# zhyever/PatchFusion

Hardware: AMD Instinct MI355X
Metric: patches/sec (DepthAnything-ViT-L PatchFusion, 4K image, P=16 tiles at N=1) (higher is better)
Workload: dtype f32; 1 GPU; Depth-Anything-vitl14 PatchFusion, 2160x3840 synthetic RGB, 4x4 regular tiling (cai_mode m1, 16 tiles), process_num=8, random-init weights (BASELINE.json configs[2] at N=1; 16 tiles per GPU); parallelism=single GPU

## Files before the change

### include/pf_hip.h

```cpp
#ifndef PF_HIP_H
#define PF_HIP_H
#include <stdint.h>

#ifdef __cplusplus
extern "C" {
#endif

#define PF_DTYPE_F32 0
#define PF_DTYPE_BF16 1

#define PF_ACT_NONE 0
#define PF_ACT_RELU 1
#define PF_ACT_GELU 2
#define PF_ACT_SOFTPLUS 3

const char* pf_last_error(void);
int pf_version(void);

typedef struct {
  const void* x; int x_ld; int B, H, W, Cin;
  const void* w; int w_rows; int Kpad;
  const float* bias; const float* scale;
  const void* res; int res_ld; const void* res2; int res2_ld;
  void* y; int y_ld; int OH, OW, Cout;
  int KH, KW, stride, pad;
  int act;
  int relu_in;
  int out_f32;
  int shuffle;
  int dtype;
  int korder;
  int batch;
  long x_bstride, w_bstride, y_bstride;
  const int* col_exp;
  const int* out_exp;
} pf_conv_params;
int pf_conv(const pf_conv_params* p, void* stream);
int pf_conv_timed(const pf_conv_params* p, int iters, float* ms, void* stream);

int pf_conv_winograd(const pf_conv_params* p, int m, const void* U, int u_rows, int u_kpad, void* V, void* M, void* stream);
int pf_conv_winograd_split3(const pf_conv_params* p, const void* U3, int u_rows, int u_kpad, void* V3, void* M, void* stream);
int pf_conv_winograd_split3_windowed(const pf_conv_params* p, const void* U3, int u_rows, int u_kpad, void* V3, void* M, long window, void* stream);
long pf_wino_f16x2_scratch_bytes(int cin, int u_rows);
int pf_conv_winograd_f16x2_supported(const pf_conv_params* p, int u_rows, int u_kpad, long window);
int pf_conv_winograd_f16x2_windowed(const pf_conv_params* p, const void* U, int u_rows, int u_kpad, void* V2, void* M, void* scratch, long window,
                                    void* stream);
int pf_conv_winograd_f16x2_windowed_ex(const pf_conv_params* p, const void* U, int u_rows, int u_kpad, void* V2, void* M, void* scratch, long window,
                                       const void* cmax_in, void* cmax_out, int cmax_out_relu, void* stream);
int pf_conv_winograd_split3_windowed_ex(const pf_conv_params* p, const void* U3, int u_rows, int u_kpad, void* V3, void* M, long window, void* cmax_out,
                                        int cmax_out_relu, void* stream);
int pf_wino_absmax(const void* x, int x_ld, long P, int C, int relu_in, void* cmax, void* stream);
int pf_gemm_f16x2_points(const pf_conv_params* p, const int* col_exp, int grid_cap, void* stream);
int pf_gemm_f16x2_points128(const pf_conv_params* p, const int* col_exp, int grid_cap, void* stream);
int pf_gemm_f16x2_points_route(const pf_conv_params* p, int cus);
int pf_gemm_f16x2_points_route_ex(const pf_conv_params* p, int cus, int maxima_given);
int pf_conv_winograd_f16x2_supported_ex(const pf_conv_params* p, int u_rows, int u_kpad, long window, int maxima_given);
int pf_gemm_f16x2(const pf_conv_params* p, void* stream);

int pf_conv_winograd_fused_supported(const pf_conv_params* p);
int pf_conv_winograd_fused(const pf_conv_params* p, const void* up, int nnb, int gs, void* stream);
int pf_conv_winograd_fused_timed(const pf_conv_params* p, const void* up, int nnb, int gs, int iters, float* ms, void* stream);

int pf_gemm_split3(const pf_conv_params* p, void* stream);
int pf_conv1x1_split3(const pf_conv_params* p, const void* w3, int w3_rows, void* stream);
int pf_gemm_split3_ex(const pf_conv_params* p, int grid_cap, void* stream);
#define PF_S3_ROUTE_TILE64 0
#define PF_S3_ROUTE_TILE128 1
#define PF_S3_ROUTE_PERSIST128 2
#define PF_S3_ROUTE_PERSIST192 3
int pf_gemm_split3_route(const pf_conv_params* p, int cus);
int pf_gemm_split3_timed(const pf_conv_params* p, int iters, float* ms, void* stream);
int pf_gemm_bf16_pp(const pf_conv_params* p, void* stream);
int pf_layernorm_split3(const float* x, int x_ld, void* y3, int y_ld, long plane, int kmajor, const float* g, const float* b, float eps,
                        long rows, int D, void* stream);
int pf_layernorm_f16x2(const float* x, int x_ld, void* y2, const int* in_exp, const float* g, const float* b, float eps, long rows, int D,
                       void* stream);
int pf_vit_attention_qkv_split3(const void* qkv, void* out3, long plane, int kmajor, int B, int S, int Hh, void* stream);
int pf_vit_attention_split3(const void* qkv3, long plane_in, void* out3, long plane_out, int kmajor, int B, int S, int Hh, void* stream);
int pf_vit_attention_split3_v2(const void* qkv3, long plane_in, void* out3, long plane_out, int kmajor, int B, int S, int Hh, int queries_per_wave,
                               int schedule, void* stream);
int pf_vit_attention_f16x2(const void* qkv2, long plane_in, const int* qk_exp, void* out, long plane_out, const int* v_exp3, int B, int S, int Hh,
                           void* stream);
int pf_vit_attention_split3_rpb(const void* qkv3, long plane_in, void* out3, long plane_out, int kmajor, int B, int S, int Hh, const float* tab,
                                int th, int tw, int queries_per_wave, void* stream);
int pf_vit_attention_rpb_bf16(const void* q, const void* k, const void* vt, void* out, int B, int S, int Sp, int Hh, const float* tab, int th, int tw,
                              void* stream);
int pf_vit_attention_rpb_bf16_lds_bytes(int S, int th, int tw);
int pf_split3(const float* x, int x_ld, void* y, int y_ld, long plane, long rows, int cols, void* stream);

int pf_patch_im2col(const float* img, int B, int H, int W, void* out, int ld, int dtype, void* stream);
int pf_patch_im2col_norm(const float* img, int B, int H, int W, int patch, const float* mean3, const float* std3, float* out, int ld, void* stream);
int pf_readout_concat(const float* x, int x_ld, int B, int S, int D, float* y, int y_ld, void* stream);
int pf_patch_im2col_norm_bf16(const float* img, int B, int H, int W, int patch, const float* mean3, const float* std3, void* out, int ld, void* stream);
int pf_readout_concat_bf16(const void* x, int x_ld, int B, int S, int D, void* y, int y_ld, void* stream);
int pf_assemble_tokens(const void* emb, void* tokens, const float* cls, const float* pos, int B, int S, int D, int dtype,
                       void* stream);
int pf_layernorm(const void* x, int x_ld, void* y, int y_ld, const float* g, const float* b, float eps,
                 int batches, int in_rows_per_batch, int in_row_offset, int out_rows_per_batch, int D,
                 int dtype, void* stream);
int pf_qkv_split(const void* qkv, int B, int S, int Hh, void* q, void* k, void* vt, int Sp, float scale,
                 int dtype, void* stream);
int pf_vit_attention(const void* q, const void* k, const void* vt, void* out, int B, int S, int Sp, int Hh,
                     int dtype, void* stream);
int pf_vit_attention_qkv(const void* qkv, void* out, int B, int S, int Hh, int dtype, void* stream);

int pf_swin_ln_partition(const void* x, int x_ld, void* xw, const float* g, const float* b, float eps,
                         int B, int H, int W, int C, int shift, int dtype, void* stream);
int pf_swin_window_attention(const void* qkv, void* out, const float* bias_table, int B, int Hp, int Wp,
                             int C, int heads, int shift, int dtype, void* stream);
int pf_swin_unpartition_add(const void* proj, const void* shortcut, int s_ld, void* y, int y_ld, int B, int H,
                            int W, int C, int shift, int dtype, void* stream);
int pf_add_rowwise(void* x, int x_ld, const float* pos, int B, int T, int C, int dtype, void* stream);

int pf_resize_bilinear(const void* x, int x_ld, int B, int H, int W, int C, void* y, int y_ld, int OH, int OW,
                       const void* add, int add_ld, int in_f32, int out_f32, int dtype, void* stream);
int pf_resize_concat(const void* const* xs, const int* lds, const int* Hs, const int* Ws, const int* Cs, int nsrc, int B,
                     void* y, int y_ld, int OH, int OW, int dtype, void* stream);
int pf_crop_resize_planar(const float* img, int C, int H, int W, const int* boxes, int P, float* out, int oh, int ow,
                          void* stream);
int pf_roi_align(const void* feat, int f_ld, int Bf, int H, int W, int C, const float* rois, int K, void* y,
                 int y_ld, int oh, int ow, float spatial_scale, int in_f32, int out_f32, int dtype, void* stream);
int pf_maxpool2(const void* x, int x_ld, int B, int H, int W, int C, void* y, int y_ld, int dtype, void* stream);
int pf_copy_channels(const void* x, int x_ld, void* y, int y_ld, long npix, int C, int in_f32, int out_f32,
                     int dtype, void* stream);
int pf_zero_u32(void* p, long n, void* stream);
int pf_resize_bilinear_ex(const void* x, int x_ld, int B, int H, int W, int C, void* y, int y_ld, int OH, int OW,
                          const void* add, int add_ld, int in_f32, int out_f32, int dtype, void* cmax, void* stream);
int pf_resize_concat_ex(const void* const* xs, const int* lds, const int* Hs, const int* Ws, const int* Cs, int nsrc, int B,
                        void* y, int y_ld, int OH, int OW, int dtype, void* cmax, void* stream);
int pf_roi_align_ex(const void* feat, int f_ld, int Bf, int H, int W, int C, const float* rois, int K, void* y,
                    int y_ld, int oh, int ow, float spatial_scale, int in_f32, int out_f32, int dtype, void* cmax, void* stream);
int pf_copy_channels_ex(const void* x, int x_ld, void* y, int y_ld, long npix, int C, int in_f32, int out_f32,
                        int dtype, void* cmax, void* stream);
int pf_pack_fusion_input(const float* cdepth, const float* fdepth, const float* crops, void* y, int B, int h, int w,
                         int dtype, void* stream);
int pf_nhwc_to_nchw_f32(const void* x, int x_ld, float* y, int B, int H, int W, int C, int in_f32, int dtype, void* stream);

int pf_attractor(const float* A, int a_ld, int n_attr, int a_stride, float a_eps, int attractor_exp, int kind_sum,
                 const float* b_prev, int hp, int wp, float* out, int B, int h, int w, int n_bins, void* stream);
int pf_seed_bin_centers(const float* x, int x_ld, float* out, long npix, int n_bins, float min_depth, float max_depth, int bounded,
                        int normalize, void* stream);
int pf_bounded_bin_centers(const float* b, float* out, long npix, int n_bins, float min_depth, float max_depth, void* stream);
int pf_logbinom_depth(const float* pt, int pt_ld, const float* centers, int hc, int wc, float* depth, int B, int h,
                      int w, int n_bins, float min_temp, float max_temp, void* stream);
int pf_bins_tail(const float* clb, int clb_ld, int rel_off, const float* emb, int he, int we, const float* w0f, const float* b0,
                 const float* w2, const float* b2, const float* centers, int hc, int wc, float* depth, int B, int H, int W, int nq,
                 float min_temp, float max_temp, void* stream);

int pf_stitch_init(float* pred, float* count, int MH, int MW, const float* depth, const float* mask, const int* yx,
                   int P, int ph, int pw, void* stream);
int pf_stitch_finish_init(float* avg, const float* pred, const float* count, long n, void* stream);
int pf_stitch_update(float* avg, float* count, int MH, int MW, const float* depth, int dh, int dw, const float* mask,
                     int y0, int x0, int ph, int pw, void* stream);
int pf_resize_nearest_f32(const float* x, int H, int W, float* y, int OH, int OW, void* stream);
int pf_resize_bilinear_f32(const float* x, int H, int W, float* y, int OH, int OW, void* stream);


int pf_u8_bicubic_to_f32(const uint8_t* src, int H, int W, int reverse_channels, float* dst, int OH, int OW, void* stream);

int pf_percentile_workspace_bytes(void);
int pf_percentiles_f32(const float* x, long n, float invalid_val, int use_invalid, const uint8_t* invalid_mask, double q0, double q1,
                       float* out2, void* workspace, void* stream);

int pf_colorize_f32(const float* depth, long n, const float* vmin_vmax, const uint8_t* lut_rgba, int N, float invalid_val,
                    int use_invalid, const uint8_t* invalid_mask, uint32_t background_rgba, uint8_t* out_rgba, void* stream);

int pf_depth_to_u16(const float* depth, long n, float scale, uint16_t* out, void* stream);

int pf_depth_metrics(const float* gt, int H, int W, const float* pred, int ph, int pw, const float* edges,
                     const uint8_t* additional_mask, float min_depth, float max_depth, int crop_y0, int crop_y1, int crop_x0, int crop_x1,
                     double* out13, void* stream);

int pf_silog_loss(const float* pred, const float* target, long n, float min_depth, float max_depth, float beta, double* ws3,
                  float* loss, void* stream);

#ifdef __cplusplus
}
#endif
#endif
```

### patchfusion_amd/_lib.py

```python
import ctypes as C
import os

import torch

_HERE = os.path.dirname(os.path.abspath(__file__))
LIB_PATH = os.environ.get("PF_LIB_PATH") or os.path.join(_HERE, "libpf_hip.so")

vp, ci, cf, cl = C.c_void_p, C.c_int, C.c_float, C.c_long


class ConvParams(C.Structure):
    _fields_ = [
        ("x", vp), ("x_ld", ci), ("B", ci), ("H", ci), ("W", ci), ("Cin", ci),
        ("w", vp), ("w_rows", ci), ("Kpad", ci),
        ("bias", vp), ("scale", vp),
        ("res", vp), ("res_ld", ci), ("res2", vp), ("res2_ld", ci),
        ("y", vp), ("y_ld", ci), ("OH", ci), ("OW", ci), ("Cout", ci),
        ("KH", ci), ("KW", ci), ("stride", ci), ("pad", ci),
        ("act", ci), ("relu_in", ci), ("out_f32", ci), ("shuffle", ci), ("dtype", ci), ("korder", ci),
        ("batch", ci), ("x_bstride", C.c_long), ("w_bstride", C.c_long), ("y_bstride", C.c_long),
        ("col_exp", vp), ("out_exp", vp),
    ]


SIGNATURES = {
    "pf_conv": [C.POINTER(ConvParams), vp],
    "pf_conv_timed": [C.POINTER(ConvParams), ci, C.POINTER(cf), vp],
    "pf_patch_im2col": [vp, ci, ci, ci, vp, ci, ci, vp],
    "pf_assemble_tokens": [vp, vp, vp, vp, ci, ci, ci, ci, vp],
    "pf_layernorm": [vp, ci, vp, ci, vp, vp, cf, ci, ci, ci, ci, ci, ci, vp],
    "pf_qkv_split": [vp, ci, ci, ci, vp, vp, vp, ci, cf, ci, vp],
    "pf_vit_attention": [vp, vp, vp, vp, ci, ci, ci, ci, ci, vp],
    "pf_vit_attention_qkv": [vp, vp, ci, ci, ci, ci, vp],
    "pf_swin_ln_partition": [vp, ci, vp, vp, vp, cf, ci, ci, ci, ci, ci, ci, vp],
    "pf_swin_window_attention": [vp, vp, vp, ci, ci, ci, ci, ci, ci, ci, vp],
    "pf_swin_unpartition_add": [vp, vp, ci, vp, ci, ci, ci, ci, ci, ci, ci, vp],
    "pf_add_rowwise": [vp, ci, vp, ci, ci, ci, ci, vp],
    "pf_resize_bilinear": [vp, ci, ci, ci, ci, ci, vp, ci, ci, ci, vp, ci, ci, ci, ci, vp],
    "pf_resize_concat": [C.POINTER(vp), C.POINTER(ci), C.POINTER(ci), C.POINTER(ci), C.POINTER(ci), ci, ci, vp, ci, ci, ci, ci, vp],
    "pf_crop_resize_planar": [vp, ci, ci, ci, vp, ci, vp, ci, ci, vp],
    "pf_roi_align": [vp, ci, ci, ci, ci, ci, vp, ci, vp, ci, ci, ci, cf, ci, ci, ci, vp],
    "pf_maxpool2": [vp, ci, ci, ci, ci, ci, vp, ci, ci, vp],
    "pf_copy_channels": [vp, ci, vp, ci, cl, ci, ci, ci, ci, vp],
    "pf_resize_bilinear_ex": [vp, ci, ci, ci, ci, ci, vp, ci, ci, ci, vp, ci, ci, ci, ci, vp, vp],
    "pf_resize_concat_ex": [C.POINTER(vp), C.POINTER(ci), C.POINTER(ci), C.POINTER(ci), C.POINTER(ci), ci, ci, vp, ci, ci, ci, ci, vp, vp],
    "pf_roi_align_ex": [vp, ci, ci, ci, ci, ci, vp, ci, vp, ci, ci, ci, cf, ci, ci, ci, vp, vp],
    "pf_copy_channels_ex": [vp, ci, vp, ci, cl, ci, ci, ci, ci, vp, vp],
    "pf_zero_u32": [vp, cl, vp],
    "pf_pack_fusion_input": [vp, vp, vp, vp, ci, ci, ci, ci, vp],
    "pf_nhwc_to_nchw_f32": [vp, ci, vp, ci, ci, ci, ci, ci, ci, vp],
    "pf_conv_winograd": [C.POINTER(ConvParams), ci, vp, ci, ci, vp, vp, vp],
    "pf_conv_winograd_split3": [C.POINTER(ConvParams), vp, ci, ci, vp, vp, vp],
    "pf_conv_winograd_split3_windowed": [C.POINTER(ConvParams), vp, ci, ci, vp, vp, C.c_long, vp],
    "pf_conv_winograd_f16x2_windowed": [C.POINTER(ConvParams), vp, ci, ci, vp, vp, vp, C.c_long, vp],
    "pf_conv_winograd_f16x2_windowed_ex": [C.POINTER(ConvParams), vp, ci, ci, vp, vp, vp, C.c_long, vp, vp, ci, vp],
    "pf_conv_winograd_split3_windowed_ex": [C.POINTER(ConvParams), vp, ci, ci, vp, vp, C.c_long, vp, ci, vp],
    "pf_wino_absmax": [vp, ci, cl, ci, ci, vp, vp],
    "pf_gemm_f16x2_points": [C.POINTER(ConvParams), vp, ci, vp],
    "pf_gemm_f16x2_points128": [C.POINTER(ConvParams), vp, ci, vp],
    "pf_gemm_f16x2": [C.POINTER(ConvParams), vp],
    "pf_gemm_split3": [C.POINTER(ConvParams), vp],
    "pf_gemm_split3_ex": [C.POINTER(ConvParams), ci, vp],
    "pf_conv1x1_split3": [C.POINTER(ConvParams), vp, ci, vp],
    "pf_gemm_split3_timed": [C.POINTER(ConvParams), ci, C.POINTER(cf), vp],
    "pf_gemm_bf16_pp": [C.POINTER(ConvParams), vp],
    "pf_split3": [vp, ci, vp, ci, cl, cl, ci, vp],
    "pf_layernorm_split3": [vp, ci, vp, ci, cl, ci, vp, vp, cf, cl, ci, vp],
    "pf_layernorm_f16x2": [vp, ci, vp, vp, vp, vp, cf, cl, ci, vp],
    "pf_vit_attention_qkv_split3": [vp, vp, cl, ci, ci, ci, ci, vp],
    "pf_vit_attention_split3": [vp, cl, vp, cl, ci, ci, ci, ci, vp],
    "pf_vit_attention_split3_v2": [vp, cl, vp, cl, ci, ci, ci, ci, ci, ci, vp],
    "pf_vit_attention_f16x2": [vp, cl, vp, vp, cl, vp, ci, ci, ci, vp],
    "pf_vit_attention_split3_rpb": [vp, cl, vp, cl, ci, ci, ci, ci, vp, ci, ci, ci, vp],
    "pf_patch_im2col_norm": [vp, ci, ci, ci, ci, vp, vp, vp, ci, vp],
    "pf_readout_concat": [vp, ci, ci, ci, ci, vp, ci, vp],
    "pf_vit_attention_rpb_bf16": [vp, vp, vp, vp, ci, ci, ci, ci, vp, ci, ci, vp],
    "pf_patch_im2col_norm_bf16": [vp, ci, ci, ci, ci, vp, vp, vp, ci, vp],
    "pf_readout_concat_bf16": [vp, ci, ci, ci, ci, vp, ci, vp],
    "pf_conv_winograd_fused": [C.POINTER(ConvParams), vp, ci, ci, vp],
    "pf_conv_winograd_fused_timed": [C.POINTER(ConvParams), vp, ci, ci, ci, C.POINTER(cf), vp],
    "pf_attractor": [vp, ci, ci, ci, cf, ci, ci, vp, ci, ci, vp, ci, ci, ci, ci, vp],
    "pf_seed_bin_centers": [vp, ci, vp, cl, ci, cf, cf, ci, ci, vp],
    "pf_bounded_bin_centers": [vp, vp, cl, ci, cf, cf, vp],
    "pf_logbinom_depth": [vp, ci, vp, ci, ci, vp, ci, ci, ci, ci, cf, cf, vp],
    "pf_bins_tail": [vp, ci, ci, vp, ci, ci, vp, vp, vp, vp, vp, ci, ci, vp, ci, ci, ci, ci, cf, cf, vp],
    "pf_stitch_init": [vp, vp, ci, ci, vp, vp, vp, ci, ci, ci, vp],
    "pf_stitch_finish_init": [vp, vp, vp, cl, vp],
    "pf_stitch_update": [vp, vp, ci, ci, vp, ci, ci, vp, ci, ci, ci, ci, vp],
    "pf_resize_nearest_f32": [vp, ci, ci, vp, ci, ci, vp],
    "pf_resize_bilinear_f32": [vp, ci, ci, vp, ci, ci, vp],
    "pf_u8_bicubic_to_f32": [vp, ci, ci, ci, vp, ci, ci, vp],
    "pf_percentiles_f32": [vp, cl, cf, ci, vp, C.c_double, C.c_double, vp, vp, vp],
    "pf_colorize_f32": [vp, cl, vp, vp, ci, cf, ci, vp, C.c_uint32, vp, vp],
    "pf_depth_to_u16": [vp, cl, cf, vp, vp],
    "pf_silog_loss": [vp, vp, cl, cf, cf, cf, vp, vp, vp],
    "pf_depth_metrics": [vp, ci, ci, vp, ci, ci, vp, vp, cf, cf, ci, ci, ci, ci, vp, vp],
}
NON_STATUS = ("pf_last_error", "pf_version", "pf_percentile_workspace_bytes", "pf_conv_winograd_fused_supported", "pf_gemm_split3_route",
              "pf_gemm_f16x2_points_route", "pf_gemm_f16x2_points_route_ex", "pf_conv_winograd_f16x2_supported_ex",
              "pf_wino_f16x2_scratch_bytes", "pf_conv_winograd_f16x2_supported", "pf_vit_attention_rpb_bf16_lds_bytes")

_lib = None


def load():
    global _lib
    if _lib is not None:
        return _lib
    if not os.path.exists(LIB_PATH):
        raise ImportError(
            f"{LIB_PATH} not found: the HIP extension is not built. Run `python __graft_entry__.py` "
            "(or `make -C patchfusion_amd/csrc`). There is no CPU fallback for the product path.")
    lib = C.CDLL(LIB_PATH)
    for name, args in SIGNATURES.items():
        fn = getattr(lib, name)
        fn.argtypes = args
        fn.restype = ci
    lib.pf_last_error.restype = C.c_char_p
    lib.pf_last_error.argtypes = []
    lib.pf_version.restype = ci
    lib.pf_version.argtypes = []
    lib.pf_percentile_workspace_bytes.restype = ci
    lib.pf_percentile_workspace_bytes.argtypes = []
    lib.pf_conv_winograd_fused_supported.restype = ci
    lib.pf_conv_winograd_fused_supported.argtypes = [C.POINTER(ConvParams)]
    lib.pf_gemm_split3_route.restype = ci
    lib.pf_gemm_split3_route.argtypes = [C.POINTER(ConvParams), ci]
    lib.pf_gemm_f16x2_points_route.restype = ci
    lib.pf_gemm_f16x2_points_route.argtypes = [C.POINTER(ConvParams), ci]
    lib.pf_gemm_f16x2_points_route_ex.restype = ci
    lib.pf_gemm_f16x2_points_route_ex.argtypes = [C.POINTER(ConvParams), ci, ci]
    lib.pf_conv_winograd_f16x2_supported_ex.restype = ci
    lib.pf_conv_winograd_f16x2_supported_ex.argtypes = [C.POINTER(ConvParams), ci, ci, C.c_long, ci]
    lib.pf_wino_f16x2_scratch_bytes.restype = C.c_long
    lib.pf_wino_f16x2_scratch_bytes.argtypes = [ci, ci]
    lib.pf_conv_winograd_f16x2_supported.restype = ci
    lib.pf_conv_winograd_f16x2_supported.argtypes = [C.POINTER(ConvParams), ci, ci, C.c_long]
    lib.pf_vit_attention_rpb_bf16_lds_bytes.restype = ci
    lib.pf_vit_attention_rpb_bf16_lds_bytes.argtypes = [ci, ci, ci]
    _lib = lib
    return lib


class PfError(RuntimeError):
    pass


def check(rc, what):
    if rc != 0:
        msg = load().pf_last_error()
        raise PfError(f"{what} failed (status {rc}): {msg.decode() if msg else ''}")
```

### patchfusion_amd/csrc/imageops.hip

```cpp
#include <atomic>
#include "pf_common.h"
#include "../../include/pf_hip.h"

namespace pf_f16x2 {
int launch_absmax(const float* x, int x_ld, long P, int C, int relu_in, unsigned* cmax, hipStream_t st);
}

namespace {

inline int grid_for(long n, int block) {
  long g = (n + block - 1) / block;
  return (int)(g > 16384 ? 16384 : (g < 1 ? 1 : g));
}
inline int ok() { return hipGetLastError() == hipSuccess ? PF_OK : PF_ERR_LAUNCH; }

struct Lerp {
  int i0, i1;
  float l0, l1;
};
__device__ __forceinline__ Lerp ac_coord(int dst, float scale, int in) {
#pragma clang fp contract(off)
  const float src = scale * dst;
  Lerp r;
  r.i0 = (int)src;
  r.i1 = r.i0 + (r.i0 < in - 1 ? 1 : 0);
  r.l1 = src - r.i0;
  r.l0 = 1.0f - r.l1;
  return r;
}
__device__ __forceinline__ float bilerp(const Lerp& ly, const Lerp& lx, float v00, float v01, float v10, float v11) {
#pragma clang fp contract(off)
  return ly.l0 * (lx.l0 * v00 + lx.l1 * v01) + ly.l1 * (lx.l0 * v10 + lx.l1 * v11);
}
inline float ac_scale(int in, int out) { return out > 1 ? (float)(in - 1) / (float)(out - 1) : 0.f; }

template <typename T>
__device__ __forceinline__ void ld8x(const void* p, long off, int f32, float (&v)[8]) {
  if (f32) load8(reinterpret_cast<const float*>(p) + off, v);
  else load8(reinterpret_cast<const T*>(p) + off, v);
}
template <typename T>
__device__ __forceinline__ void st8x(void* p, long off, int f32, const float (&v)[8]) {
  if (f32) store8(reinterpret_cast<float*>(p) + off, v);
  else store8(reinterpret_cast<T*>(p) + off, v);
}

template <typename T>
__global__ void resize_bilinear_kernel(const void* __restrict__ x, int x_ld, int B, int H, int W, int C, void* __restrict__ y,
                                       int y_ld, int OH, int OW, const void* __restrict__ add, int add_ld, int in_f32,
                                       int out_f32, float sh, float sw) {
  const int cv = C >> 3;
  const int n = OW * cv;
  for (int row = blockIdx.y; row < B * OH; row += gridDim.y) {
  const int b = row / OH, oy = row - b * OH;
  const Lerp ly = ac_coord(oy, sh, H);
  const long r0 = ((long)b * H + ly.i0) * W, r1 = ((long)b * H + ly.i1) * W;
  const long orow = (long)row * OW;
  for (int i = blockIdx.x * blockDim.x + threadIdx.x; i < n; i += gridDim.x * blockDim.x) {
    const int ox = i / cv, v = i - ox * cv;
    const Lerp lx = ac_coord(ox, sw, W);
    float v00[8], v01[8], v10[8], v11[8], o[8];
    ld8x<T>(x, (r0 + lx.i0) * x_ld + v * 8, in_f32, v00);
    ld8x<T>(x, (r0 + lx.i1) * x_ld + v * 8, in_f32, v01);
    ld8x<T>(x, (r1 + lx.i0) * x_ld + v * 8, in_f32, v10);
    ld8x<T>(x, (r1 + lx.i1) * x_ld + v * 8, in_f32, v11);
#pragma unroll
    for (int e = 0; e < 8; ++e) o[e] = bilerp(ly, lx, v00[e], v01[e], v10[e], v11[e]);
    const long pix = orow + ox;
    if (add) {
      float a[8];
      ld8x<T>(add, pix * add_ld + v * 8, out_f32, a);
#pragma unroll
      for (int e = 0; e < 8; ++e) o[e] = a[e] + o[e];
    }
    st8x<T>(y, pix * y_ld + v * 8, out_f32, o);
  }
  }
}

struct ResizeSrc {
  const void* x;
  int ld, H, W, C;
  float sh, sw;
};
template <typename T>
__global__ void resize_concat_kernel(ResizeSrc s0, ResizeSrc s1, ResizeSrc s2, int nsrc, int B, void* __restrict__ y, int y_ld,
                                     int OH, int OW) {
  for (int row = blockIdx.y; row < B * OH; row += gridDim.y) {
    const int b = row / OH, oy = row - b * OH;
    const long orow = (long)row * OW;
    int coff = 0;
    for (int si = 0; si < nsrc; ++si) {
      const ResizeSrc& s = si == 0 ? s0 : (si == 1 ? s1 : s2);
      const int cv = s.C >> 3;
      const int n = OW * cv;
      const Lerp ly = ac_coord(oy, s.sh, s.H);
      const long r0 = ((long)b * s.H + ly.i0) * s.W, r1 = ((long)b * s.H + ly.i1) * s.W;
      for (int i = blockIdx.x * blockDim.x + threadIdx.x; i < n; i += gridDim.x * blockDim.x) {
        const int ox = i / cv, v = i - ox * cv;
        const Lerp lx = ac_coord(ox, s.sw, s.W);
        float v00[8], v01[8], v10[8], v11[8], o[8];
        ld8x<T>(s.x, (r0 + lx.i0) * s.ld + v * 8, 0, v00);
        ld8x<T>(s.x, (r0 + lx.i1) * s.ld + v * 8, 0, v01);
        ld8x<T>(s.x, (r1 + lx.i0) * s.ld + v * 8, 0, v10);
        ld8x<T>(s.x, (r1 + lx.i1) * s.ld + v * 8, 0, v11);
#pragma unroll
        for (int e = 0; e < 8; ++e) o[e] = bilerp(ly, lx, v00[e], v01[e], v10[e], v11[e]);
        st8x<T>(y, (orow + ox) * y_ld + coff + v * 8, 0, o);
      }
      coff += s.C;
    }
  }
}

__device__ __forceinline__ int first_dst(int c, float scale, int out) {
  if (c <= 0) return 0;
  if (scale <= 0.f) return out;
  int o = (int)((float)c / scale);
  o = o < 0 ? 0 : (o > out ? out : o);
  while (o > 0 && (int)(scale * (o - 1)) >= c) --o;
  while (o < out && (int)(scale * o) < c) ++o;
  return o;
}

template <typename T>
__device__ __forceinline__ void ldv(const T* p, float (&v)[16 / sizeof(T)]) {
  if constexpr (sizeof(T) == 4) load4(p, v);
  else load8(p, v);
}
template <typename T>
__device__ __forceinline__ void stv(T* p, const float (&v)[16 / sizeof(T)]) {
  if constexpr (sizeof(T) == 4) store4(p, v[0], v[1], v[2], v[3]);
  else store8(p, v);
}

template <int N>
struct CmaxRun {
  unsigned m[N];
  int v = -1;
  __device__ __forceinline__ void flush(unsigned* sm) {
    if (v < 0) return;
#pragma unroll
    for (int e = 0; e < N; ++e)
      if (m[e]) atomicMax(&sm[v * N + e], m[e]);
  }
  __device__ __forceinline__ void take(int vec, const float (&o)[N], unsigned* sm) {
    if (vec != v) {
      flush(sm);
      v = vec;
#pragma unroll
      for (int e = 0; e < N; ++e) m[e] = 0u;
    }
#pragma unroll
    for (int e = 0; e < N; ++e) m[e] = max(m[e], __float_as_uint(o[e]) & 0x7fffffffu);
  }
};
__device__ __forceinline__ void cmax_merge_block(const unsigned* sm, int C, unsigned* cmax) {
  for (int i = threadIdx.x; i < C; i += blockDim.x)
    if (sm[i] > cmax[i]) atomicMax(&cmax[i], sm[i]);
}

constexpr int RESIZE_RPB = 8;
template <typename T, bool CMAX = false>
__global__ void resize_src_kernel(ResizeSrc s0, ResizeSrc s1, ResizeSrc s2, int nsrc, int B, int Hmax, void* __restrict__ yv, int y_ld, int OH,
                                  int OW, const void* __restrict__ addv, int add_ld, int Wmax, int rpb, unsigned* __restrict__ cmax) {
  constexpr int N = 16 / sizeof(T);
  extern __shared__ __attribute__((aligned(16))) char resize_lds[];
  int2* rowrange = reinterpret_cast<int2*>(resize_lds);
  int2* colrange = reinterpret_cast<int2*>(resize_lds + RESIZE_RPB * 8);
  float2* wx = reinterpret_cast<float2*>(resize_lds + RESIZE_RPB * 8 + (size_t)Wmax * 8);
  unsigned* csm = reinterpret_cast<unsigned*>(resize_lds + RESIZE_RPB * 8 + (size_t)Wmax * 8 + (size_t)OW * 8);
  const int ctot = s0.C + (nsrc > 1 ? s1.C : 0) + (nsrc > 2 ? s2.C : 0);
  if constexpr (CMAX) {
    for (int i = threadIdx.x; i < ctot; i += blockDim.x) csm[i] = 0u;
  }
  T* __restrict__ y = reinterpret_cast<T*>(yv);
  const T* __restrict__ add = reinterpret_cast<const T*>(addv);
  const int tid = threadIdx.x, nthr = blockDim.x * gridDim.x, gtid = blockIdx.x * blockDim.x + tid;
  const int gpi = (Hmax + rpb - 1) / rpb;
  int coff = 0;
  for (int si = 0; si < nsrc; ++si) {
    const ResizeSrc& s = si == 0 ? s0 : (si == 1 ? s1 : s2);
    __syncthreads();
    for (int c = tid; c < s.W; c += blockDim.x) colrange[c] = make_int2(first_dst(c, s.sw, OW), first_dst(c + 1, s.sw, OW));
    for (int ox = tid; ox < OW; ox += blockDim.x) {
      const Lerp lx = ac_coord(ox, s.sw, s.W);
      wx[ox] = make_float2(lx.l0, lx.l1);
    }
    const T* __restrict__ x = reinterpret_cast<const T*>(s.x);
    const int cv = s.C / N, n = s.W * cv;
    const float inv_cv = 1.0f / (float)cv;
    CmaxRun<N> run;
    for (int g = blockIdx.y; g < B * gpi; g += gridDim.y) {
      const int b = g / gpi, rbeg = (g - b * gpi) * rpb;
      const int rend = rbeg + rpb < s.H ? rbeg + rpb : s.H;
      __syncthreads();
      if (tid < rpb) rowrange[tid] = make_int2(first_dst(rbeg + tid, s.sh, OH), first_dst(rbeg + tid + 1, s.sh, OH));
      __syncthreads();
      if (rbeg >= rend) continue;
      for (int i = gtid; i < n; i += nthr) {
        int c = (int)(((float)i + 0.5f) * inv_cv);
        int v = i - c * cv;
        if (v < 0) { --c; v += cv; } else if (v >= cv) { ++c; v -= cv; }
        const int2 rg = colrange[c];
        if (rg.x >= rg.y) continue;
        const long o0 = (long)c * s.ld + v * N, o1 = (long)(c + (c < s.W - 1 ? 1 : 0)) * s.ld + v * N;
        const T* __restrict__ rowp = x + ((long)b * s.H + rbeg) * s.W * s.ld;
        float v00[N], v01[N], v10[N], v11[N];
        ldv<T>(rowp + o0, v00);
        ldv<T>(rowp + o1, v01);
        for (int r = rbeg; r < rend; ++r) {
          if (r < s.H - 1) {
            rowp += (long)s.W * s.ld;
            ldv<T>(rowp + o0, v10);
            ldv<T>(rowp + o1, v11);
          } else {
#pragma unroll
            for (int e = 0; e < N; ++e) { v10[e] = v00[e]; v11[e] = v01[e]; }
          }
          const int2 rr = rowrange[r - rbeg];
          for (int oy = rr.x; oy < rr.y; ++oy) {
            const Lerp ly = ac_coord(oy, s.sh, s.H);
            const long pix0 = ((long)b * OH + oy) * OW;
            T* __restrict__ yp = y + (pix0 + rg.x) * y_ld + coff + v * N;
            for (int ox = rg.x; ox < rg.y; ++ox, yp += y_ld) {
              const float2 w = wx[ox];
              Lerp lx;
              lx.l0 = w.x;
              lx.l1 = w.y;
              float o[N];
#pragma unroll
              for (int e = 0; e < N; ++e) o[e] = bilerp(ly, lx, v00[e], v01[e], v10[e], v11[e]);
              if (add) {
                float a[N];
                ldv<T>(add + (pix0 + ox) * add_ld + v * N, a);
#pragma unroll
                for (int e = 0; e < N; ++e) o[e] = a[e] + o[e];
              }
              stv<T>(yp, o);
              if constexpr (CMAX) run.take(v, o, csm + coff);
            }
          }
#pragma unroll
          for (int e = 0; e < N; ++e) { v00[e] = v10[e]; v01[e] = v11[e]; }
        }
      }
    }
    if constexpr (CMAX) run.flush(csm + coff);
    coff += s.C;
  }
  if constexpr (CMAX) {
    __syncthreads();
    cmax_merge_block(csm, ctot, cmax);
  }
}

__global__ void crop_resize_planar_kernel(const float* __restrict__ img, int C, int H, int W, const int* __restrict__ boxes, int P,
                                          float* __restrict__ out, int oh, int ow) {
  const long total = (long)P * C * oh * ow;
  for (long i = (long)blockIdx.x * blockDim.x + threadIdx.x; i < total; i += (long)gridDim.x * blockDim.x) {
    const int ox = (int)(i % ow);
    const int oy = (int)((i / ow) % oh);
    const int c = (int)((i / ((long)ow * oh)) % C);
    const int p = (int)(i / ((long)ow * oh * C));
    const int x0 = boxes[p * 4 + 0], y0 = boxes[p * 4 + 1], bw = boxes[p * 4 + 2] - x0, bh = boxes[p * 4 + 3] - y0;
    const float sh = oh > 1 ? (float)(bh - 1) / (float)(oh - 1) : 0.f;
    const float sw = ow > 1 ? (float)(bw - 1) / (float)(ow - 1) : 0.f;
    const Lerp ly = ac_coord(oy, sh, bh), lx = ac_coord(ox, sw, bw);
    const float* src = img + (long)c * H * W;
    const float v00 = src[(long)(y0 + ly.i0) * W + x0 + lx.i0], v01 = src[(long)(y0 + ly.i0) * W + x0 + lx.i1];
    const float v10 = src[(long)(y0 + ly.i1) * W + x0 + lx.i0], v11 = src[(long)(y0 + ly.i1) * W + x0 + lx.i1];
    out[i] = ly.l0 * (lx.l0 * v00 + lx.l1 * v01) + ly.l1 * (lx.l0 * v10 + lx.l1 * v11);
  }
}

template <typename T, bool CMAX = false>
__global__ __launch_bounds__(256) void roi_align_kernel(const void* __restrict__ feat, int f_ld, int Bf, int H, int W, int C,
                                                        const float* __restrict__ rois, int K, void* __restrict__ y, int y_ld, int oh, int ow,
                                                        float scale, int in_f32, int out_f32, unsigned* __restrict__ cmax) {
  extern __shared__ unsigned roi_csm[];
  CmaxRun<8> run;
  if constexpr (CMAX) {
    for (int i = threadIdx.x; i < C; i += blockDim.x) roi_csm[i] = 0u;
    __syncthreads();
  }
  const int cv = (C + 7) >> 3;
  const int k = blockIdx.x / oh, ph = blockIdx.x - k * oh;
  const float* r = rois + k * 5;
  const int b = (int)r[0];
  const float start_w = __fsub_rn(__fmul_rn(r[1], scale), 0.5f), start_h = __fsub_rn(__fmul_rn(r[2], scale), 0.5f);
  const float end_w = __fsub_rn(__fmul_rn(r[3], scale), 0.5f), end_h = __fsub_rn(__fmul_rn(r[4], scale), 0.5f);
  const float roi_w = __fsub_rn(end_w, start_w), roi_h = __fsub_rn(end_h, start_h);
  const float bin_h = __fdiv_rn(roi_h, (float)oh), bin_w = __fdiv_rn(roi_w, (float)ow);
  const int gh = (int)ceilf(__fdiv_rn(roi_h, (float)oh)), gw = (int)ceilf(__fdiv_rn(roi_w, (float)ow));
  const float count = (float)max(gh * gw, 1);
  const long base = (long)b * H * W;
  const long row_pix = ((long)k * oh + ph) * ow;
  const float y_row = __fadd_rn(start_h, __fmul_rn((float)ph, bin_h));
  constexpr int RUN = 4;
  const int groups = (ow + RUN - 1) / RUN;
  const int items = groups * cv;
  for (int i = threadIdx.x; i < items; i += blockDim.x) {
    const int pg = i / cv, v = i - pg * cv;
    int c_yl = -1, c_xl = -1, c_yh = -1, c_xh = -1;
    float v1[8], v2[8], v3[8], v4[8];
#pragma unroll
    for (int q = 0; q < RUN; ++q) {
      const int pw = pg * RUN + q;
      if (pw >= ow) break;
      const float x_col = __fadd_rn(start_w, __fmul_rn((float)pw, bin_w));
      float acc[8];
#pragma unroll
      for (int e = 0; e < 8; ++e) acc[e] = 0.f;
      for (int iy = 0; iy < gh; ++iy) {
        const float yy = __fadd_rn(y_row, __fdiv_rn(__fmul_rn((float)iy + 0.5f, bin_h), (float)gh));
        for (int ix = 0; ix < gw; ++ix) {
          float xx = __fadd_rn(x_col, __fdiv_rn(__fmul_rn((float)ix + 0.5f, bin_w), (float)gw));
          float y2 = yy;
          if (y2 < -1.0f || y2 > (float)H || xx < -1.0f || xx > (float)W) continue;
          if (y2 <= 0.f) y2 = 0.f;
          if (xx <= 0.f) xx = 0.f;
          int yl = (int)y2, xl = (int)xx, yh, xh;
          if (yl >= H - 1) { yh = yl = H - 1; y2 = (float)yl; } else yh = yl + 1;
          if (xl >= W - 1) { xh = xl = W - 1; xx = (float)xl; } else xh = xl + 1;
          const float ly = y2 - yl, lx = xx - xl, hy = 1.f - ly, hx = 1.f - lx;
          const float w1 = hy * hx, w2 = hy * lx, w3 = ly * hx, w4 = ly * lx;
          if (yl != c_yl || xl != c_xl || yh != c_yh || xh != c_xh) {
            ld8x<T>(feat, (base + (long)yl * W + xl) * f_ld + v * 8, in_f32, v1);
            ld8x<T>(feat, (base + (long)yl * W + xh) * f_ld + v * 8, in_f32, v2);
            ld8x<T>(feat, (base + (long)yh * W + xl) * f_ld + v * 8, in_f32, v3);
            ld8x<T>(feat, (base + (long)yh * W + xh) * f_ld + v * 8, in_f32, v4);
            c_yl = yl; c_xl = xl; c_yh = yh; c_xh = xh;
          }
#pragma unroll
          for (int e = 0; e < 8; ++e) acc[e] += w1 * v1[e] + w2 * v2[e] + w3 * v3[e] + w4 * v4[e];
        }
      }
      if (count != 1.0f) {
#pragma unroll
        for (int e = 0; e < 8; ++e) acc[e] /= count;
      }
      st8x<T>(y, (row_pix + pw) * y_ld + v * 8, out_f32, acc);
      if constexpr (CMAX) run.take(v, acc, roi_csm);
    }
  }
  if constexpr (CMAX) {
    run.flush(roi_csm);
    __syncthreads();
    cmax_merge_block(roi_csm, C, cmax);
  }
}

__global__ void roi_align_scalar_kernel(const float* __restrict__ feat, int Bf, int H, int W, const float* __restrict__ rois, int K,
                                        float* __restrict__ y, int oh, int ow, float scale) {
  const long total = (long)K * oh * ow;
  for (long i = (long)blockIdx.x * blockDim.x + threadIdx.x; i < total; i += (long)gridDim.x * blockDim.x) {
    const int pw = (int)(i % ow);
    const int ph = (int)((i / ow) % oh);
    const int k = (int)(i / ((long)ow * oh));
    const float* r = rois + k * 5;
    const int b = (int)r[0];
    const float start_w = __fsub_rn(__fmul_rn(r[1], scale), 0.5f), start_h = __fsub_rn(__fmul_rn(r[2], scale), 0.5f);
    const float end_w = __fsub_rn(__fmul_rn(r[3], scale), 0.5f), end_h = __fsub_rn(__fmul_rn(r[4], scale), 0.5f);
    const float roi_w = __fsub_rn(end_w, start_w), roi_h = __fsub_rn(end_h, start_h);
    const float bin_h = __fdiv_rn(roi_h, (float)oh), bin_w = __fdiv_rn(roi_w, (float)ow);
    const int gh = (int)ceilf(__fdiv_rn(roi_h, (float)oh)), gw = (int)ceilf(__fdiv_rn(roi_w, (float)ow));
    const float count = (float)max(gh * gw, 1);
    const float* src = feat + (long)b * H * W;
    float acc = 0.f;
    for (int iy = 0; iy < gh; ++iy) {
      const float yy0 = __fadd_rn(__fadd_rn(start_h, __fmul_rn((float)ph, bin_h)), __fdiv_rn(__fmul_rn((float)iy + 0.5f, bin_h), (float)gh));
      for (int ix = 0; ix < gw; ++ix) {
        float xx = __fadd_rn(__fadd_rn(start_w, __fmul_rn((float)pw, bin_w)), __fdiv_rn(__fmul_rn((float)ix + 0.5f, bin_w), (float)gw));
        float y2 = yy0;
        if (y2 < -1.0f || y2 > (float)H || xx < -1.0f || xx > (float)W) continue;
        if (y2 <= 0.f) y2 = 0.f;
        if (xx <= 0.f) xx = 0.f;
        int yl = (int)y2, xl = (int)xx, yh, xh;
        if (yl >= H - 1) { yh = yl = H - 1; y2 = (float)yl; } else yh = yl + 1;
        if (xl >= W - 1) { xh = xl = W - 1; xx = (float)xl; } else xh = xl + 1;
        const float ly = y2 - yl, lx = xx - xl, hy = 1.f - ly, hx = 1.f - lx;
        acc += hy * hx * src[(long)yl * W + xl] + hy * lx * src[(long)yl * W + xh] + ly * hx * src[(long)yh * W + xl] + ly * lx * src[(long)yh * W + xh];
      }
    }
    y[i] = acc / count;
  }
}
// ... 696 lines not shown
```

### patchfusion_amd/csrc/pf_common.h

```cpp
#pragma once
#include <hip/hip_runtime.h>
#include <stdint.h>

typedef __attribute__((ext_vector_type(4))) float f32x4;
typedef __attribute__((ext_vector_type(8))) __bf16 bf16x8;
typedef __attribute__((ext_vector_type(8))) _Float16 f16x8;
typedef uint16_t bf16_t;

#define PF_WAVE 64

__device__ __forceinline__ float bf2f(bf16_t h) { return __uint_as_float(((uint32_t)h) << 16); }
__device__ __forceinline__ bf16_t f2bf(float f) {
  uint32_t u = __float_as_uint(f);
  u += 0x7fffu + ((u >> 16) & 1u);
  return (bf16_t)(u >> 16);
}

__device__ __forceinline__ uint32_t cvt_pk_bf16(float lo, float hi) {
  uint32_t r;
  asm("v_cvt_pk_bf16_f32 %0, %1, %2" : "=v"(r) : "v"(lo), "v"(hi));
  return r;
}

template <typename T> struct Elem;
template <> struct Elem<float> {
  static constexpr int VEC = 4;
  __device__ static __forceinline__ float ld(const float* p) { return *p; }
  __device__ static __forceinline__ void st(float* p, float v) { *p = v; }
};
template <> struct Elem<bf16_t> {
  static constexpr int VEC = 8;
  __device__ static __forceinline__ float ld(const bf16_t* p) { return bf2f(*p); }
  __device__ static __forceinline__ void st(bf16_t* p, float v) { *p = f2bf(v); }
};

__device__ __forceinline__ void load8(const float* p, float (&v)[8]) {
  float4 a = *reinterpret_cast<const float4*>(p), b = *reinterpret_cast<const float4*>(p + 4);
  v[0] = a.x; v[1] = a.y; v[2] = a.z; v[3] = a.w; v[4] = b.x; v[5] = b.y; v[6] = b.z; v[7] = b.w;
}
__device__ __forceinline__ void load8(const bf16_t* p, float (&v)[8]) {
  uint4 a = *reinterpret_cast<const uint4*>(p);
  uint32_t w[4] = {a.x, a.y, a.z, a.w};
#pragma unroll
  for (int i = 0; i < 4; ++i) {
    v[2 * i] = __uint_as_float(w[i] << 16);
    v[2 * i + 1] = __uint_as_float(w[i] & 0xffff0000u);
  }
}
__device__ __forceinline__ void store8(float* p, const float (&v)[8]) {
  *reinterpret_cast<float4*>(p) = make_float4(v[0], v[1], v[2], v[3]);
  *reinterpret_cast<float4*>(p + 4) = make_float4(v[4], v[5], v[6], v[7]);
}
__device__ __forceinline__ void store8(bf16_t* p, const float (&v)[8]) {
  uint4 a;
  a.x = cvt_pk_bf16(v[0], v[1]);
  a.y = cvt_pk_bf16(v[2], v[3]);
  a.z = cvt_pk_bf16(v[4], v[5]);
  a.w = cvt_pk_bf16(v[6], v[7]);
  *reinterpret_cast<uint4*>(p) = a;
}
__device__ __forceinline__ void store4(float* p, float a, float b, float c, float d) {
  *reinterpret_cast<float4*>(p) = make_float4(a, b, c, d);
}
__device__ __forceinline__ void store4(bf16_t* p, float a, float b, float c, float d) {
  uint2 r;
  r.x = (uint32_t)f2bf(a) | ((uint32_t)f2bf(b) << 16);
  r.y = (uint32_t)f2bf(c) | ((uint32_t)f2bf(d) << 16);
  *reinterpret_cast<uint2*>(p) = r;
}

__device__ __forceinline__ void split3_pair(float a, float b, uint32_t& h, uint32_t& m, uint32_t& l) {
#pragma clang fp contract(off)
  h = cvt_pk_bf16(a, b);
  const float ra = a - __uint_as_float(h << 16), rb = b - __uint_as_float(h & 0xffff0000u);
  m = cvt_pk_bf16(ra, rb);
  l = cvt_pk_bf16(ra - __uint_as_float(m << 16), rb - __uint_as_float(m & 0xffff0000u));
}
__device__ __forceinline__ void store_split3(bf16_t* y, long plane, const float (&v)[4]) {
  uint32_t h0, m0, l0, h1, m1, l1;
  split3_pair(v[0], v[1], h0, m0, l0);
  split3_pair(v[2], v[3], h1, m1, l1);
  *reinterpret_cast<uint2*>(y) = make_uint2(h0, h1);
  *reinterpret_cast<uint2*>(y + plane) = make_uint2(m0, m1);
  *reinterpret_cast<uint2*>(y + 2 * plane) = make_uint2(l0, l1);
}

__device__ __forceinline__ long split3_at(long row, int col, int ld, long kmaj_rows) {
  return kmaj_rows ? ((long)(col >> 5) * kmaj_rows + row) * 32 + (col & 31) : row * ld + col;
}

__device__ __forceinline__ void load4(const float* p, float (&v)[4]) {
  float4 a = *reinterpret_cast<const float4*>(p);
  v[0] = a.x; v[1] = a.y; v[2] = a.z; v[3] = a.w;
}
__device__ __forceinline__ void load4(const bf16_t* p, float (&v)[4]) {
  uint2 a = *reinterpret_cast<const uint2*>(p);
  v[0] = __uint_as_float(a.x << 16); v[1] = __uint_as_float(a.x & 0xffff0000u);
  v[2] = __uint_as_float(a.y << 16); v[3] = __uint_as_float(a.y & 0xffff0000u);
}

__device__ __forceinline__ float gelu_erf(float x) {
#ifdef PF_GELU_OCML
  return 0.5f * x * (1.0f + erff(x * 0.70710678118654752440f));
#else
  const float a = fminf(fabsf(x) * 0.70710678118654752440f, 4.0f);
  float p = -2.8146364456915762e-06f;
  p = __builtin_fmaf(p, a, 5.093829895486124e-05f);
  p = __builtin_fmaf(p, a, -0.00036259577609598637f);
  p = __builtin_fmaf(p, a, 0.0010585421696305275f);
  p = __builtin_fmaf(p, a, 0.0016202160622924566f);
  p = __builtin_fmaf(p, a, -0.029034368693828583f);
  p = __builtin_fmaf(p, a, 0.14880506694316864f);
  p = __builtin_fmaf(p, a, 0.9183712005615234f);
  p = __builtin_fmaf(p, a, 1.6279088258743286f);
  const float e = 1.0f - __builtin_amdgcn_exp2f(-(p * a));
  return 0.5f * x * (1.0f + copysignf(e, x));
#endif
}
__device__ __forceinline__ float softplus20(float x) { return x > 20.0f ? x : log1pf(expf(x)); }

__device__ __forceinline__ float wave_sum(float v) {
#pragma unroll
  for (int o = 32; o > 0; o >>= 1) v += __shfl_xor(v, o, 64);
  return v;
}
__device__ __forceinline__ float wave_max(float v) {
#pragma unroll
  for (int o = 32; o > 0; o >>= 1) v = fmaxf(v, __shfl_xor(v, o, 64));
  return v;
}

__device__ __forceinline__ int xcd_remap(int bid, int nblocks) {
  const int NX = 8;
  int q = nblocks / NX, r = nblocks % NX;
  int xcd = bid % NX, idx = bid / NX;
  int base = (xcd < r) ? xcd * (q + 1) : r * (q + 1) + (xcd - r) * q;
  return base + idx;
}

#define PF_OK 0
#define PF_ERR_ARG 1
#define PF_ERR_LAUNCH 2
```

### patchfusion_amd/csrc/wino_f16x2.hip

```cpp
#include <climits>
#include "pf_common.h"
#include "../../include/pf_hip.h"

namespace {

__device__ __forceinline__ int clog2(float a) {
  int e;
  const float f = frexpf(a, &e);
  return f == 0.5f ? e - 1 : e;
}
__device__ __forceinline__ int chan_exp(unsigned mb) { return (mb == 0u || mb >= 0x7f800000u) ? 0 : clog2(__uint_as_float(mb)) - 8; }

__device__ __forceinline__ uint32_t pack_h2(_Float16 a, _Float16 b) {
  return (uint32_t)__builtin_bit_cast(uint16_t, a) | ((uint32_t)__builtin_bit_cast(uint16_t, b) << 16);
}

__global__ __launch_bounds__(256) void wino_absmax_kernel(const float* __restrict__ x, int x_ld, long P, int C, int relu_in, long R,
                                                          unsigned* __restrict__ cmax) {
  extern __shared__ unsigned sm[];
  const int cv = C >> 2;
  for (int i = threadIdx.x; i < C; i += blockDim.x) sm[i] = 0u;
  __syncthreads();
  const long idx = (long)blockIdx.x * blockDim.x + threadIdx.x;
  if (idx < (long)cv * R) {
    const int c4 = (int)(idx % cv);
    long r = idx / cv;
    const float* xp = x + c4 * 4;
    uint32_t m[4] = {0u, 0u, 0u, 0u};
    auto take = [&](float4 v) __attribute__((always_inline)) {
      if (relu_in) { v.x = fmaxf(v.x, 0.f); v.y = fmaxf(v.y, 0.f); v.z = fmaxf(v.z, 0.f); v.w = fmaxf(v.w, 0.f); }
      m[0] = max(m[0], __float_as_uint(v.x) & 0x7fffffffu);
      m[1] = max(m[1], __float_as_uint(v.y) & 0x7fffffffu);
      m[2] = max(m[2], __float_as_uint(v.z) & 0x7fffffffu);
      m[3] = max(m[3], __float_as_uint(v.w) & 0x7fffffffu);
    };
    for (; r + 3 * R < P; r += 4 * R) {
      const float4 a = *reinterpret_cast<const float4*>(xp + r * x_ld);
      const float4 b = *reinterpret_cast<const float4*>(xp + (r + R) * x_ld);
      const float4 c = *reinterpret_cast<const float4*>(xp + (r + 2 * R) * x_ld);
      const float4 d = *reinterpret_cast<const float4*>(xp + (r + 3 * R) * x_ld);
      take(a); take(b); take(c); take(d);
    }
    for (; r < P; r += R) take(*reinterpret_cast<const float4*>(xp + r * x_ld));
#pragma unroll
    for (int e = 0; e < 4; ++e)
      if (m[e]) atomicMax(&sm[c4 * 4 + e], m[e]);
  }
  __syncthreads();
  for (int i = threadIdx.x; i < C; i += blockDim.x)
    if (sm[i]) atomicMax(&cmax[i], sm[i]);
}

__global__ __launch_bounds__(256) void wino_u_split_kernel(const float* __restrict__ U, int rows, int C, int npts, const unsigned* __restrict__ cmax,
                                                           uint16_t* __restrict__ U2, int* __restrict__ fexp) {
  const int wv = (int)blockIdx.x * 4 + (int)(threadIdx.x >> 6), lane = threadIdx.x & 63;
  if (wv >= npts * rows) return;
  const int pt = wv / rows, n = wv - pt * rows;
  const float* u = U + ((long)pt * rows + n) * C;
  int mx = INT_MIN;
  for (int c = lane; c < C; c += 64) {
    const float a = fabsf(u[c]);
    if (a != 0.f && a < INFINITY) mx = max(mx, clog2(a) + chan_exp(cmax[c]));
  }
#pragma unroll
  for (int o = 32; o >= 1; o >>= 1) mx = max(mx, __shfl_xor(mx, o));
  const int f = mx == INT_MIN ? 0 : mx - 15;
  const size_t plane = (size_t)npts * C * rows;
  for (int c = lane; c < C; c += 64) {
    const float v = ldexpf(u[c], chan_exp(cmax[c]) - f);
    const _Float16 h = (_Float16)v, l = (_Float16)(v - (float)h);
    const size_t o = (((size_t)pt * (C >> 5) + (c >> 5)) * rows + n) * 32 + (c & 31);
    U2[o] = __builtin_bit_cast(uint16_t, h);
    U2[o + plane] = __builtin_bit_cast(uint16_t, l);
  }
  if (lane == 0) fexp[pt * rows + n] = f;
}

__device__ __forceinline__ void bt6(float (&d)[6]) {
  const float o0 = 4.f * d[0] - 5.f * d[2] + d[4];
  const float o1 = -4.f * (d[1] + d[2]) + d[3] + d[4];
  const float o2 = 4.f * (d[1] - d[2]) - d[3] + d[4];
  const float o3 = -2.f * d[1] - d[2] + 2.f * d[3] + d[4];
  const float o4 = 2.f * d[1] - d[2] - 2.f * d[3] + d[4];
  const float o5 = 4.f * d[1] - 5.f * d[3] + d[5];
  d[0] = o0; d[1] = o1; d[2] = o2; d[3] = o3; d[4] = o4; d[5] = o5;
}

__global__ __launch_bounds__(512) void wino_input_f16x2_kernel(const float* __restrict__ x, int x_ld, int B, int H, int W, int C, int relu_in,
                                                               const unsigned* __restrict__ cmax, uint16_t* __restrict__ V, int TH, int TW, long total,
                                                               long tile0, long T) {
  constexpr int MT = 4, A = 6;
  const int nkc = C >> 5;
  for (long idx = (long)blockIdx.x * blockDim.x + threadIdx.x; idx < total; idx += (long)gridDim.x * blockDim.x) {
    const long w64 = idx >> 6;
    const long tile = (w64 / nkc) * 8 + ((idx >> 3) & 7);
    const int c4 = (int)(w64 % nkc) * 8 + (int)(idx & 7);
    if (tile >= T) continue;
    const long gt = tile + tile0;
    const int tx = (int)(gt % TW), ty = (int)((gt / TW) % TH), b = (int)(gt / ((long)TW * TH));
    const uint4 mb = *reinterpret_cast<const uint4*>(cmax + c4 * 4);
    const int ne[4] = {-chan_exp(mb.x), -chan_exp(mb.y), -chan_exp(mb.z), -chan_exp(mb.w)};
    float d[A][A][4];
#pragma unroll
    for (int i = 0; i < A; ++i) {
      const int y = ty * MT - 1 + i;
#pragma unroll
      for (int j = 0; j < A; ++j) {
        const int xx = tx * MT - 1 + j;
        float4 v = make_float4(0.f, 0.f, 0.f, 0.f);
        if ((unsigned)y < (unsigned)H && (unsigned)xx < (unsigned)W)
          v = *reinterpret_cast<const float4*>(x + (((long)b * H + y) * W + xx) * x_ld + c4 * 4);
        if (relu_in) { v.x = fmaxf(v.x, 0.f); v.y = fmaxf(v.y, 0.f); v.z = fmaxf(v.z, 0.f); v.w = fmaxf(v.w, 0.f); }
        d[i][j][0] = v.x; d[i][j][1] = v.y; d[i][j][2] = v.z; d[i][j][3] = v.w;
      }
    }
#pragma unroll
    for (int e = 0; e < 4; ++e) {
#pragma unroll
      for (int j = 0; j < A; ++j) {
        float col[A];
#pragma unroll
        for (int i = 0; i < A; ++i) col[i] = d[i][j][e];
        bt6(col);
#pragma unroll
        for (int i = 0; i < A; ++i) d[i][j][e] = col[i];
      }
#pragma unroll
      for (int i = 0; i < A; ++i) {
        float row[A];
#pragma unroll
        for (int j = 0; j < A; ++j) row[j] = d[i][j][e];
        bt6(row);
#pragma unroll
        for (int j = 0; j < A; ++j) d[i][j][e] = row[j];
      }
    }
    const size_t plane = (size_t)T * C;
    uint16_t* o = V + ((size_t)(c4 >> 3) * T + tile) * 32 + (c4 & 7) * 4;
#pragma unroll
    for (int i = 0; i < A; ++i)
#pragma unroll
      for (int j = 0; j < A; ++j) {
        _Float16 h[4], l[4];
#pragma unroll
        for (int e = 0; e < 4; ++e) {
          const float v = ldexpf(d[i][j][e], ne[e]);
          h[e] = (_Float16)v;
          l[e] = (_Float16)(v - (float)h[e]);
        }
        uint16_t* q = o + (size_t)(i * A + j) * plane;
        *reinterpret_cast<uint2*>(q) = make_uint2(pack_h2(h[0], h[1]), pack_h2(h[2], h[3]));
        *reinterpret_cast<uint2*>(q + (size_t)A * A * plane) = make_uint2(pack_h2(l[0], l[1]), pack_h2(l[2], l[3]));
      }
  }
}

}

namespace pf_f16x2 {

int launch_absmax(const float* x, int x_ld, long P, int C, int relu_in, unsigned* cmax, hipStream_t st) {
  const int cv = C >> 2;
  long R = (256L * 2048L) / cv;
  if (R < 1) R = 1;
  if (R > P) R = P;
  const long threads = (long)cv * R;
  hipLaunchKernelGGL(wino_absmax_kernel, dim3((unsigned)((threads + 255) / 256)), dim3(256), (size_t)C * 4, st, x, x_ld, P, C, relu_in, R, cmax);
  return hipGetLastError() == hipSuccess ? PF_OK : PF_ERR_LAUNCH;
}

int launch_u_split(const float* U, int rows, int C, const unsigned* cmax, void* U2, int* fexp, hipStream_t st) {
  const long waves = 36L * rows;
  hipLaunchKernelGGL(wino_u_split_kernel, dim3((unsigned)((waves + 3) / 4)), dim3(256), 0, st, U, rows, C, 36, cmax, static_cast<uint16_t*>(U2), fexp);
  return hipGetLastError() == hipSuccess ? PF_OK : PF_ERR_LAUNCH;
}

int launch_input(const float* x, int x_ld, int B, int H, int W, int C, int relu_in, const unsigned* cmax, void* V, int TH, int TW, long tile0, long T,
                 hipStream_t st) {
  const long nin = ((T + 7) / 8) * 8 * (C / 4);
  hipLaunchKernelGGL(wino_input_f16x2_kernel, dim3((unsigned)((nin + 255) / 256)), dim3(256), 0, st, x, x_ld, B, H, W, C, relu_in, cmax,
                     static_cast<uint16_t*>(V), TH, TW, nin, tile0, T);
  return hipGetLastError() == hipSuccess ? PF_OK : PF_ERR_LAUNCH;
}

}
```

### patchfusion_amd/csrc/winograd.hip

```cpp
#include <mutex>
#include "pf_common.h"
#include "../../include/pf_hip.h"

namespace pf_f16x2 {
int launch_absmax(const float* x, int x_ld, long P, int C, int relu_in, unsigned* cmax, hipStream_t st);
int launch_u_split(const float* U, int rows, int C, const unsigned* cmax, void* U2, int* fexp, hipStream_t st);
int launch_input(const float* x, int x_ld, int B, int H, int W, int C, int relu_in, const unsigned* cmax, void* V, int TH, int TW, long tile0, long T,
                 hipStream_t st);
int launch_output_cmax(const float* M, const pf_conv_params* p, int TH, int TW, long t0, long T, unsigned* cmax, int cmax_relu, hipStream_t st);
}

namespace {

#define ST(s) reinterpret_cast<hipStream_t>(s)

template <int MT> struct Wino;
template <> struct Wino<2> {
  __device__ static __forceinline__ void bt(float (&d)[4]) {
    const float o0 = d[0] - d[2], o1 = d[1] + d[2], o2 = d[2] - d[1], o3 = d[1] - d[3];
    d[0] = o0; d[1] = o1; d[2] = o2; d[3] = o3;
  }
  __device__ static __forceinline__ void at(const float (&m)[4], float (&o)[2]) {
    o[0] = m[0] + m[1] + m[2];
    o[1] = m[1] - m[2] - m[3];
  }
};
template <> struct Wino<4> {
  __device__ static __forceinline__ void bt(float (&d)[6]) {
    const float o0 = 4.f * d[0] - 5.f * d[2] + d[4];
    const float o1 = -4.f * (d[1] + d[2]) + d[3] + d[4];
    const float o2 = 4.f * (d[1] - d[2]) - d[3] + d[4];
    const float o3 = -2.f * d[1] - d[2] + 2.f * d[3] + d[4];
    const float o4 = 2.f * d[1] - d[2] - 2.f * d[3] + d[4];
    const float o5 = 4.f * d[1] - 5.f * d[3] + d[5];
    d[0] = o0; d[1] = o1; d[2] = o2; d[3] = o3; d[4] = o4; d[5] = o5;
  }
  __device__ static __forceinline__ void at(const float (&m)[6], float (&o)[4]) {
    const float s12 = m[1] + m[2], d12 = m[1] - m[2], s34 = m[3] + m[4], d34 = m[3] - m[4];
    o[0] = m[0] + s12 + s34;
    o[1] = d12 + 2.f * d34;
    o[2] = s12 + 4.f * s34;
    o[3] = d12 + 8.f * d34 + m[5];
  }
};

template <int MT, bool SPLIT = false>
__global__ __launch_bounds__(512) void wino_input_kernel(const float* __restrict__ x, int x_ld, int B, int H, int W, int C, int relu_in,
                                                         float* __restrict__ V, int TH, int TW, long total, long tile0, long T) {
  constexpr int A = MT + 2;
  const int cv = C >> 2;
  for (long idx = (long)blockIdx.x * blockDim.x + threadIdx.x; idx < total; idx += (long)gridDim.x * blockDim.x) {
  int c4;
  long tile;
  if constexpr (SPLIT) {
    const int nkc = C >> 5;
    const long w64 = idx >> 6;
    tile = (w64 / nkc) * 8 + ((idx >> 3) & 7);
    c4 = (int)(w64 % nkc) * 8 + (int)(idx & 7);
    if (tile >= T) continue;
  } else {
    if (idx >= T * cv) continue;
    c4 = (int)(idx % cv);
    tile = idx / cv;
  }
  const long gt = tile + tile0;
  const int tx = (int)(gt % TW), ty = (int)((gt / TW) % TH), b = (int)(gt / ((long)TW * TH));
  float d[A][A][4];
#pragma unroll
  for (int i = 0; i < A; ++i) {
    const int y = ty * MT - 1 + i;
#pragma unroll
    for (int j = 0; j < A; ++j) {
      const int xx = tx * MT - 1 + j;
      float4 v = make_float4(0.f, 0.f, 0.f, 0.f);
      if ((unsigned)y < (unsigned)H && (unsigned)xx < (unsigned)W)
        v = *reinterpret_cast<const float4*>(x + (((long)b * H + y) * W + xx) * x_ld + c4 * 4);
      if (relu_in) { v.x = fmaxf(v.x, 0.f); v.y = fmaxf(v.y, 0.f); v.z = fmaxf(v.z, 0.f); v.w = fmaxf(v.w, 0.f); }
      d[i][j][0] = v.x; d[i][j][1] = v.y; d[i][j][2] = v.z; d[i][j][3] = v.w;
    }
  }
#pragma unroll
  for (int e = 0; e < 4; ++e) {
#pragma unroll
    for (int j = 0; j < A; ++j) {
      float col[A];
#pragma unroll
      for (int i = 0; i < A; ++i) col[i] = d[i][j][e];
      Wino<MT>::bt(col);
#pragma unroll
      for (int i = 0; i < A; ++i) d[i][j][e] = col[i];
    }
#pragma unroll
    for (int i = 0; i < A; ++i) {
      float row[A];
#pragma unroll
      for (int j = 0; j < A; ++j) row[j] = d[i][j][e];
      Wino<MT>::bt(row);
#pragma unroll
      for (int j = 0; j < A; ++j) d[i][j][e] = row[j];
    }
  }
  const size_t plane = (size_t)T * C;
  if constexpr (SPLIT) {
    bf16_t* o = reinterpret_cast<bf16_t*>(V) + ((size_t)(c4 >> 3) * T + tile) * 32 + (c4 & 7) * 4;
#pragma unroll
    for (int i = 0; i < A; ++i)
#pragma unroll
      for (int j = 0; j < A; ++j) store_split3(o + (size_t)(i * A + j) * plane, (long)(A * A) * (long)plane, d[i][j]);
  } else {
    float* o = V + (size_t)tile * C + c4 * 4;
#pragma unroll
    for (int i = 0; i < A; ++i)
#pragma unroll
      for (int j = 0; j < A; ++j)
        *reinterpret_cast<float4*>(o + (size_t)(i * A + j) * plane) = make_float4(d[i][j][0], d[i][j][1], d[i][j][2], d[i][j][3]);
  }
  }
}

template <int MT>
__global__ __launch_bounds__(512) void wino_output_kernel(const float* __restrict__ M, int N, const float* __restrict__ bias, int relu,
                                                          const float* __restrict__ res, int res_ld, const float* __restrict__ res2,
                                                          int res2_ld, float* __restrict__ y, int y_ld, int B, int H, int W, int TH,
                                                          int TW, long tile0, long T) {
  constexpr int A = MT + 2;
  const int nv = N >> 2;
  for (long idx = (long)blockIdx.x * blockDim.x + threadIdx.x; idx < T * nv; idx += (long)gridDim.x * blockDim.x) {
  const int n4 = (int)(idx % nv);
  const long tile = idx / nv;
  const long gt = tile + tile0;
  const int tx = (int)(gt % TW), ty = (int)((gt / TW) % TH), b = (int)(gt / ((long)TW * TH));
  const size_t plane = (size_t)T * N;
  const float* m = M + (size_t)tile * N + n4 * 4;
  float t[MT][A][4];
#pragma unroll
  for (int j = 0; j < A; ++j) {
    float col[4][A];
#pragma unroll
    for (int i = 0; i < A; ++i) {
      const float4 v = *reinterpret_cast<const float4*>(m + (size_t)(i * A + j) * plane);
      col[0][i] = v.x; col[1][i] = v.y; col[2][i] = v.z; col[3][i] = v.w;
    }
#pragma unroll
    for (int e = 0; e < 4; ++e) {
      float o[MT];
      Wino<MT>::at(col[e], o);
#pragma unroll
      for (int p = 0; p < MT; ++p) t[p][j][e] = o[p];
    }
  }
  float4 bv = make_float4(0.f, 0.f, 0.f, 0.f);
  if (bias) bv = *reinterpret_cast<const float4*>(bias + n4 * 4);
  const float be[4] = {bv.x, bv.y, bv.z, bv.w};
#pragma unroll
  for (int p = 0; p < MT; ++p) {
    const int oy = ty * MT + p;
    float r[4][MT];
#pragma unroll
    for (int e = 0; e < 4; ++e) {
      float row[A];
#pragma unroll
      for (int j = 0; j < A; ++j) row[j] = t[p][j][e];
      Wino<MT>::at(row, r[e]);
    }
    if (oy >= H) continue;
#pragma unroll
    for (int q = 0; q < MT; ++q) {
      const int ox = tx * MT + q;
      if (ox >= W) continue;
      const long pix = ((long)b * H + oy) * W + ox;
      float v[4];
#pragma unroll
      for (int e = 0; e < 4; ++e) {
        v[e] = r[e][q] + be[e];
        if (relu) v[e] = fmaxf(v[e], 0.f);
      }
      if (res) {
        const float4 a = *reinterpret_cast<const float4*>(res + pix * res_ld + n4 * 4);
        v[0] += a.x; v[1] += a.y; v[2] += a.z; v[3] += a.w;
      }
      if (res2) {
        const float4 a = *reinterpret_cast<const float4*>(res2 + pix * res2_ld + n4 * 4);
        v[0] += a.x; v[1] += a.y; v[2] += a.z; v[3] += a.w;
      }
      *reinterpret_cast<float4*>(y + pix * y_ld + n4 * 4) = make_float4(v[0], v[1], v[2], v[3]);
    }
  }
  }
}

inline int launch_ok() { return hipGetLastError() == hipSuccess ? PF_OK : PF_ERR_LAUNCH; }

template <int MT>
int run(const pf_conv_params* p, const float* U, int u_rows, int u_kpad, float* V, float* M, hipStream_t st) {
  constexpr int A = MT + 2;
  const int TH = (p->H + MT - 1) / MT, TW = (p->W + MT - 1) / MT;
  const long T = (long)p->B * TH * TW;
  if (T > 0x7fffffffL) return PF_ERR_ARG;
  const long nin = T * (p->Cin / 4), nout = T * (p->Cout / 4);
  hipLaunchKernelGGL(wino_input_kernel<MT>, dim3((unsigned)((nin + 255) / 256)), dim3(256), 0, st, static_cast<const float*>(p->x), p->x_ld,
                     p->B, p->H, p->W, p->Cin, p->relu_in, V, TH, TW, nin, 0L, T);
  if (launch_ok() != PF_OK) return PF_ERR_LAUNCH;
  pf_conv_params q = {};
  q.x_ld = p->Cin; q.B = 1; q.H = 1; q.W = (int)T; q.Cin = p->Cin;
  q.w_rows = u_rows; q.Kpad = u_kpad;
  q.y_ld = p->Cout; q.OH = 1; q.OW = (int)T; q.Cout = p->Cout;
  q.KH = q.KW = 1; q.stride = 1; q.pad = 0; q.act = PF_ACT_NONE; q.shuffle = 1; q.dtype = PF_DTYPE_F32; q.korder = 0;
  q.x = V; q.w = U; q.y = M;
  q.batch = A * A;
  q.x_bstride = T * p->Cin; q.w_bstride = (long)u_rows * u_kpad; q.y_bstride = T * p->Cout;
  const int rc = pf_conv(&q, st);
  if (rc != PF_OK) return rc;
  hipLaunchKernelGGL(wino_output_kernel<MT>, dim3((unsigned)((nout + 255) / 256)), dim3(256), 0, st, M, p->Cout, p->bias,
                     p->act == PF_ACT_RELU ? 1 : 0, static_cast<const float*>(p->res), p->res_ld, static_cast<const float*>(p->res2),
                     p->res2_ld, static_cast<float*>(p->y), p->y_ld, p->B, p->H, p->W, TH, TW, 0L, T);
  return launch_ok();
}

hipEvent_t gemm_token() {
  static hipEvent_t ev[64] = {};
  static std::once_flag once[64];
  int dev = 0;
  hipGetDevice(&dev);
  std::call_once(once[dev & 63], [&] { hipEventCreateWithFlags(&ev[dev & 63], hipEventDisableTiming); });
  return ev[dev & 63];
}

struct W3Switches { int tgrid = 0, cap = 0; bool token = false; };
const W3Switches& w3_switches() {
  static W3Switches sw;
  static std::once_flag once;
  std::call_once(once, [] {
    if (const char* s = getenv("PF_W3_TGRID")) sw.tgrid = atoi(s);
    if (const char* s = getenv("PF_W3_GRID")) sw.cap = atoi(s);
    if (const char* s = getenv("PF_W3_TOKEN")) sw.token = s[0] == '1';
  });
  return sw;
}

bool windows_alias(const pf_conv_params* p) {
  const char* xa = static_cast<const char*>(p->x);
  const char* ya = static_cast<const char*>(p->y);
  const long px = (long)p->B * p->H * p->W;
  const long xb = (px - 1) * p->x_ld * 4 + (long)p->Cin * 4, yb = (px - 1) * p->y_ld * 4 + (long)p->Cout * 4;
  if (!(xa < ya + yb && ya < xa + xb)) return false;
  const long d = (long)(ya - xa);
  if (p->x_ld != p->y_ld || p->x_ld <= 0 || d % 4) return true;
  long r = (d / 4) % p->x_ld;
  if (r < 0) r += p->x_ld;
  return !(r >= p->Cin && r + p->Cout <= p->x_ld);
}

int run_split3(const pf_conv_params* p, const void* U3, int u_rows, int u_kpad, void* V3, float* M, long window, hipStream_t st,
               unsigned* cmax_out = nullptr, int cmax_relu = 0) {
  constexpr int MT = 4, A = 6;
  const int TH = (p->H + MT - 1) / MT, TW = (p->W + MT - 1) / MT;
  const long Tall = (long)p->B * TH * TW;
  if (Tall > 0x7fffffffL) return PF_ERR_ARG;
  if (window <= 0 || window > Tall) window = Tall;
  const W3Switches& sw = w3_switches();
  const int tgrid = sw.tgrid, cap = sw.cap;
  hipEvent_t tok = sw.token ? gemm_token() : nullptr;
  if (window < Tall && windows_alias(p)) return PF_ERR_ARG;
  if (cmax_out && hipMemsetAsync(cmax_out, 0, (size_t)p->Cout * 4, st) != hipSuccess) return PF_ERR_LAUNCH;
  for (long t0 = 0; t0 < Tall; t0 += window) {
    const long T = Tall - t0 < window ? Tall - t0 : window;
    const long nin = ((T + 7) / 8) * 8 * (p->Cin / 4), nout = T * (p->Cout / 4);
    const bool resident = tgrid > 0 && nin > (long)tgrid * 512 * 4;
    const dim3 gin = resident ? dim3((unsigned)tgrid) : dim3((unsigned)((nin + 255) / 256)), bin = resident ? dim3(512) : dim3(256);
    hipLaunchKernelGGL((wino_input_kernel<MT, true>), gin, bin, 0, st, static_cast<const float*>(p->x), p->x_ld,
                       p->B, p->H, p->W, p->Cin, p->relu_in, static_cast<float*>(V3), TH, TW, nin, t0, T);
    if (launch_ok() != PF_OK) return PF_ERR_LAUNCH;
    pf_conv_params q = {};
    q.x_ld = p->Cin; q.B = 1; q.H = 1; q.W = (int)T; q.Cin = p->Cin;
    q.w_rows = u_rows; q.Kpad = u_kpad;
    q.y_ld = p->Cout; q.OH = 1; q.OW = (int)T; q.Cout = p->Cout;
    q.KH = q.KW = 1; q.stride = 1; q.pad = 0; q.act = PF_ACT_NONE; q.shuffle = 1; q.dtype = PF_DTYPE_BF16; q.out_f32 = 1;
    q.x = V3; q.w = U3; q.y = M;
    q.korder = 6;
    q.batch = A * A;
    q.x_bstride = (long)A * A * T * p->Cin;
    q.w_bstride = (long)A * A * u_rows * u_kpad;
    if (tok) hipStreamWaitEvent(st, tok, 0);
    const int rc = pf_gemm_split3_ex(&q, cap, st);
    if (rc != PF_OK) return rc;
    if (tok) hipEventRecord(tok, st);
    const bool resident_out = tgrid > 0 && nout > (long)tgrid * 512 * 4;
    if (cmax_out) {
      const int rc2 = pf_f16x2::launch_output_cmax(M, p, TH, TW, t0, T, cmax_out, cmax_relu, st);
      if (rc2 != PF_OK) return rc2;
    } else
    hipLaunchKernelGGL(wino_output_kernel<MT>, resident_out ? dim3((unsigned)tgrid) : dim3((unsigned)((nout + 255) / 256)), resident_out ? dim3(512) : dim3(256), 0, st, M,
                       p->Cout, p->bias, p->act == PF_ACT_RELU ? 1 : 0, static_cast<const float*>(p->res), p->res_ld, static_cast<const float*>(p->res2),
                       p->res2_ld, static_cast<float*>(p->y), p->y_ld, p->B, p->H, p->W, TH, TW, t0, T);
    if (!cmax_out && launch_ok() != PF_OK) return PF_ERR_LAUNCH;
  }
  return PF_OK;
}

struct F16x2Scratch { void* u2; int* fexp; unsigned* cmax; };
inline size_t align256(size_t b) { return (b + 255) & ~(size_t)255; }
F16x2Scratch f16x2_scratch(void* base, int cin, int u_rows) {
  char* b = static_cast<char*>(base);
  const size_t u2 = align256((size_t)2 * 36 * u_rows * cin * 2), fe = align256((size_t)36 * u_rows * 4);
  return {b, reinterpret_cast<int*>(b + u2), reinterpret_cast<unsigned*>(b + u2 + fe)};
}

pf_conv_params f16x2_points_params(const pf_conv_params* p, const void* U2, int u_rows, void* V2, float* M, long T) {
  constexpr int A = 6;
  pf_conv_params q = {};
  q.x_ld = p->Cin; q.B = 1; q.H = 1; q.W = (int)T; q.Cin = p->Cin;
  q.w_rows = u_rows; q.Kpad = p->Cin;
  q.y_ld = p->Cout; q.OH = 1; q.OW = (int)T; q.Cout = p->Cout;
  q.KH = q.KW = 1; q.stride = 1; q.pad = 0; q.act = PF_ACT_NONE; q.shuffle = 1; q.dtype = PF_DTYPE_BF16; q.out_f32 = 1;
  q.x = V2; q.w = U2; q.y = M;
  q.korder = 6;
  q.batch = A * A;
  q.x_bstride = (long)A * A * T * p->Cin;
  q.w_bstride = (long)A * A * u_rows * p->Cin;
  return q;
}

int f16x2_layer_route(const pf_conv_params* p, int u_rows, bool maxima_given = false) {
  const long T = (long)p->B * ((p->H + 3) / 4) * ((p->W + 3) / 4);
  if (T > 0x7fffffffL) return -1;
  int dev = 0, cus = 0;
  if (hipGetDevice(&dev) != hipSuccess || hipDeviceGetAttribute(&cus, hipDeviceAttributeMultiprocessorCount, dev) != hipSuccess || cus <= 0) cus = 256;
  pf_conv_params q = f16x2_points_params(p, p->x, u_rows, const_cast<void*>(p->x), static_cast<float*>(p->y), T);
  return pf_gemm_f16x2_points_route_ex(&q, cus, maxima_given ? 1 : 0);
}

int run_f16x2(const pf_conv_params* p, const float* U, int u_rows, void* V2, float* M, void* scratch, long window, hipStream_t st,
              const unsigned* cmax_in = nullptr, unsigned* cmax_out = nullptr, int cmax_relu = 0) {
  constexpr int MT = 4;
  const bool t128 = f16x2_layer_route(p, u_rows, cmax_in != nullptr) == PF_S3_ROUTE_PERSIST128;
  const int TH = (p->H + MT - 1) / MT, TW = (p->W + MT - 1) / MT;
  const long Tall = (long)p->B * TH * TW;
  if (Tall > 0x7fffffffL) return PF_ERR_ARG;
  if (window <= 0 || window > Tall) window = Tall;
  if (window < Tall && windows_alias(p)) return PF_ERR_ARG;
  const F16x2Scratch sc = f16x2_scratch(scratch, p->Cin, u_rows);
  const float* x = static_cast<const float*>(p->x);
  int rc = PF_OK;
  const unsigned* cmax = cmax_in;
  if (!cmax) {
    if (hipMemsetAsync(sc.cmax, 0, (size_t)p->Cin * 4, st) != hipSuccess) return PF_ERR_LAUNCH;
    rc = pf_f16x2::launch_absmax(x, p->x_ld, (long)p->B * p->H * p->W, p->Cin, p->relu_in, sc.cmax, st);
    if (rc != PF_OK) return rc;
    cmax = sc.cmax;
  }
  if (cmax_out && hipMemsetAsync(cmax_out, 0, (size_t)p->Cout * 4, st) != hipSuccess) return PF_ERR_LAUNCH;
  rc = pf_f16x2::launch_u_split(U, u_rows, p->Cin, cmax, sc.u2, sc.fexp, st);
  if (rc != PF_OK) return rc;
  for (long t0 = 0; t0 < Tall; t0 += window) {
    const long T = Tall - t0 < window ? Tall - t0 : window;
    const long nout = T * (p->Cout / 4);
    rc = pf_f16x2::launch_input(x, p->x_ld, p->B, p->H, p->W, p->Cin, p->relu_in, cmax, V2, TH, TW, t0, T, st);
    if (rc != PF_OK) return rc;
    const pf_conv_params q = f16x2_points_params(p, sc.u2, u_rows, V2, M, T);
    rc = t128 ? pf_gemm_f16x2_points128(&q, sc.fexp, 0, st) : pf_gemm_f16x2_points(&q, sc.fexp, 0, st);
    if (rc != PF_OK) return rc;
    if (cmax_out) {
      rc = pf_f16x2::launch_output_cmax(M, p, TH, TW, t0, T, cmax_out, cmax_relu, st);
      if (rc != PF_OK) return rc;
      continue;
    }
    hipLaunchKernelGGL(wino_output_kernel<MT>, dim3((unsigned)((nout + 255) / 256)), dim3(256), 0, st, M, p->Cout, p->bias, p->act == PF_ACT_RELU ? 1 : 0,
                       static_cast<const float*>(p->res), p->res_ld, static_cast<const float*>(p->res2), p->res2_ld, static_cast<float*>(p->y), p->y_ld,
                       p->B, p->H, p->W, TH, TW, t0, T);
    if (launch_ok() != PF_OK) return PF_ERR_LAUNCH;
  }
  return PF_OK;
}

bool f16x2_args_ok(const pf_conv_params* p, int u_rows, int u_kpad, long window) {
  if (!p || !p->x || !p->y || window < 0 || (window > 0 && window % 8)) return false;
  if (p->dtype != PF_DTYPE_F32 || p->KH != 3 || p->KW != 3 || p->stride != 1 || p->pad != 1 || p->shuffle > 1 || p->scale) return false;
  if (p->OH != p->H || p->OW != p->W || p->Cin % 32 || p->Cout % 8 || p->Cin <= 0 || p->Cout <= 0 || p->Cin > 8192) return false;
  if (p->act != PF_ACT_NONE && p->act != PF_ACT_RELU) return false;
  return u_rows >= p->Cout && u_rows % 16 == 0 && u_kpad == p->Cin;
}

}

extern "C" long pf_wino_f16x2_scratch_bytes(int cin, int u_rows) {
  if (cin <= 0 || u_rows <= 0) return 0;
  return (long)(align256((size_t)2 * 36 * u_rows * cin * 2) + align256((size_t)36 * u_rows * 4) + align256((size_t)cin * 4));
}

extern "C" int pf_conv_winograd_f16x2_supported(const pf_conv_params* p, int u_rows, int u_kpad, long window) {
  if (!f16x2_args_ok(p, u_rows, u_kpad, window)) return 0;
  return f16x2_layer_route(p, u_rows) >= 0 ? 1 : 0;
}

extern "C" int pf_conv_winograd_f16x2_supported_ex(const pf_conv_params* p, int u_rows, int u_kpad, long window, int maxima_given) {
  if (!f16x2_args_ok(p, u_rows, u_kpad, window)) return 0;
  return f16x2_layer_route(p, u_rows, maxima_given != 0) >= 0 ? 1 : 0;
}

extern "C" int pf_conv_winograd_f16x2_windowed(const pf_conv_params* p, const void* U, int u_rows, int u_kpad, void* V2, void* M, void* scratch,
                                               long window, void* stream) {
  if (!U || !V2 || !M || !scratch || !f16x2_args_ok(p, u_rows, u_kpad, window)) return PF_ERR_ARG;
  return run_f16x2(p, static_cast<const float*>(U), u_rows, V2, static_cast<float*>(M), scratch, window, ST(stream));
}

extern "C" int pf_conv_winograd_f16x2_windowed_ex(const pf_conv_params* p, const void* U, int u_rows, int u_kpad, void* V2, void* M, void* scratch,
                                                  long window, const void* cmax_in, void* cmax_out, int cmax_out_relu, void* stream) {
  if (!U || !V2 || !M || !scratch || !f16x2_args_ok(p, u_rows, u_kpad, window) || (cmax_in && cmax_in == cmax_out)) return PF_ERR_ARG;
  return run_f16x2(p, static_cast<const float*>(U), u_rows, V2, static_cast<float*>(M), scratch, window, ST(stream),
                   static_cast<const unsigned*>(cmax_in), static_cast<unsigned*>(cmax_out), cmax_out_relu);
}

extern "C" int pf_wino_absmax(const void* x, int x_ld, long P, int C, int relu_in, void* cmax, void* stream) {
  if (!x || !cmax || P <= 0 || C <= 0 || C % 4 || x_ld < C || x_ld % 4) return PF_ERR_ARG;
  return pf_f16x2::launch_absmax(static_cast<const float*>(x), x_ld, P, C, relu_in, static_cast<unsigned*>(cmax), ST(stream));
}

extern "C" int pf_conv_winograd_split3(const pf_conv_params* p, const void* U3, int u_rows, int u_kpad, void* V3, void* M, void* stream) {
  if (!p || !U3 || !V3 || !M || !p->x || !p->y) return PF_ERR_ARG;
  if (p->dtype != PF_DTYPE_F32 || p->KH != 3 || p->KW != 3 || p->stride != 1 || p->pad != 1 || p->shuffle > 1 || p->scale) return PF_ERR_ARG;
  if (p->OH != p->H || p->OW != p->W || p->Cin % 32 || p->Cout % 8 || p->Cin <= 0 || p->Cout <= 0) return PF_ERR_ARG;
  if (p->act != PF_ACT_NONE && p->act != PF_ACT_RELU) return PF_ERR_ARG;
  if (u_rows < p->Cout || u_kpad != p->Cin) return PF_ERR_ARG;
  return run_split3(p, U3, u_rows, u_kpad, V3, static_cast<float*>(M), 0, ST(stream));
}

extern "C" int pf_conv_winograd_split3_windowed(const pf_conv_params* p, const void* U3, int u_rows, int u_kpad, void* V3, void* M, long window, void* stream) {
  if (!p || !U3 || !V3 || !M || !p->x || !p->y || window < 0 || (window > 0 && window % 8)) return PF_ERR_ARG;
  if (p->dtype != PF_DTYPE_F32 || p->KH != 3 || p->KW != 3 || p->stride != 1 || p->pad != 1 || p->shuffle > 1 || p->scale) return PF_ERR_ARG;
  if (p->OH != p->H || p->OW != p->W || p->Cin % 32 || p->Cout % 8 || p->Cin <= 0 || p->Cout <= 0) return PF_ERR_ARG;
  if (p->act != PF_ACT_NONE && p->act != PF_ACT_RELU) return PF_ERR_ARG;
  if (u_rows < p->Cout || u_kpad != p->Cin) return PF_ERR_ARG;
  return run_split3(p, U3, u_rows, u_kpad, V3, static_cast<float*>(M), window, ST(stream));
}

extern "C" int pf_conv_winograd_split3_windowed_ex(const pf_conv_params* p, const void* U3, int u_rows, int u_kpad, void* V3, void* M, long window,
                                                   void* cmax_out, int cmax_out_relu, void* stream) {
  if (!p || !U3 || !V3 || !M || !p->x || !p->y || window < 0 || (window > 0 && window % 8)) return PF_ERR_ARG;
  if (p->dtype != PF_DTYPE_F32 || p->KH != 3 || p->KW != 3 || p->stride != 1 || p->pad != 1 || p->shuffle > 1 || p->scale) return PF_ERR_ARG;
  if (p->OH != p->H || p->OW != p->W || p->Cin % 32 || p->Cout % 8 || p->Cin <= 0 || p->Cout <= 0) return PF_ERR_ARG;
  if (p->act != PF_ACT_NONE && p->act != PF_ACT_RELU) return PF_ERR_ARG;
  if (u_rows < p->Cout || u_kpad != p->Cin) return PF_ERR_ARG;
  return run_split3(p, U3, u_rows, u_kpad, V3, static_cast<float*>(M), window, ST(stream), static_cast<unsigned*>(cmax_out), cmax_out_relu);
}

extern "C" int pf_conv_winograd(const pf_conv_params* p, int m, const void* U, int u_rows, int u_kpad, void* V, void* M, void* stream) {
  if (!p || !U || !V || !M || !p->x || !p->y) return PF_ERR_ARG;
  if (p->dtype != PF_DTYPE_F32 || p->KH != 3 || p->KW != 3 || p->stride != 1 || p->pad != 1 || p->shuffle > 1 || p->scale) return PF_ERR_ARG;
  if (p->OH != p->H || p->OW != p->W || p->Cin % 32 || p->Cout % 8 || p->Cin <= 0 || p->Cout <= 0) return PF_ERR_ARG;
  if (p->act != PF_ACT_NONE && p->act != PF_ACT_RELU) return PF_ERR_ARG;
  if (u_rows < p->Cout || u_kpad < p->Cin || u_kpad % 32) return PF_ERR_ARG;
  if (m == 2) return run<2>(p, static_cast<const float*>(U), u_rows, u_kpad, static_cast<float*>(V), static_cast<float*>(M), ST(stream));
  if (m == 4) return run<4>(p, static_cast<const float*>(U), u_rows, u_kpad, static_cast<float*>(V), static_cast<float*>(M), ST(stream));
  return PF_ERR_ARG;
}
```

### patchfusion_amd/engine.py

```python
import math

import torch

from . import packing as pk
from .config import pyramid_sizes
from .spec import DPT_ARCH, VIT_ARCH, branch_channels

F32 = torch.float32


def linear_split3_enabled():
    import os
    return os.environ.get("PF_LINEAR_SPLIT3", "1") != "0"


def vit_f16x2_enabled(crops):
    import os
    v = os.environ.get("PF_VIT_F16X2", "1")
    return v == "2" or (v != "0" and crops)


def vit_attn_f16x2_enabled():
    import os
    v = os.environ.get("PF_VIT_ATTN_F16X2", "1")
# ... 223 lines not shown
        B = img.shape[0]
        T, S, D = self.th * self.tw, self.th * self.tw + 1, self.D
        col = ops.empty((B * T, 592), dt, dev)
        ops.patch_im2col(img, col)
        emb = ops.empty((B * T, D), dt, dev)
        ops.conv(col, self.pe, emb)
        tok = ops.empty((B, S, D), dt, dev)
        ops.assemble_tokens(emb, tok, self.cls, self.pos)
        x = tok.view(B * S, D)
        if taps is not None:
            taps["vit_tokens_in"] = tok.clone()
        feats = []
        if self.split3:
            if pk.split3_kmajor_enabled():
                hbuf, att, mid = (ops.empty((3, n // 32, B * S, 32), torch.bfloat16, dev) for n in (D, D, 4 * D))
            else:
                hbuf, att, mid = (ops.empty((3, B * S, n), torch.bfloat16, dev) for n in (D, D, 4 * D))
            qkv = ops.empty((3, B * S, 3 * D), torch.bfloat16, dev) if attention_split3_enabled() else ops.empty((B * S, 3 * D), dt, dev)
            if self.f16x2:
                hbuf, mid = (ops.empty((2, n // 32, B * S, 32), torch.float16, dev) for n in (D, 4 * D))
            if self.attn_f16x2:
                qkv = ops.empty((2, B * S, 3 * D), torch.float16, dev)
                if self.proj_f16x2:
                    att = ops.empty((2, D // 32, B * S, 32), torch.float16, dev)
        else:
            hbuf = ops.empty((B * S, D), dt, dev)
            qkv = ops.empty((B * S, 3 * D), dt, dev)
            att = ops.empty((B * S, D), dt, dev)
            mid = ops.empty((B * S, 4 * D), dt, dev)
        for i, blk in enumerate(self.blocks):
            if self.f16x2:
                ops.layernorm_f16x2(x, hbuf, blk["n1"][0], blk["n1"][1], 1e-6, blk["qkv"].in_exp)
                if self.attn_f16x2:
                    ops.conv_f16x2(hbuf, blk["qkv"], qkv, out_exp=blk["attn"].out_exp)
                    if self.proj_f16x2:
                        ops.vit_attention_f16x2(qkv, att, B, S, self.heads, blk["attn"].qk_exp)
                        ops.conv_f16x2(att, blk["proj"], x, res=x)
                    else:
                        ops.vit_attention_f16x2(qkv, att, B, S, self.heads, blk["attn"].qk_exp, v_exp=blk["attn"].v_exp)
                        ops.conv_split3(att, blk["proj"], x, res=x)
                else:
                    ops.conv_f16x2(hbuf, blk["qkv"], qkv)
                    ops.vit_attention(qkv, att, B, S, self.heads)
                    ops.conv_split3(att, blk["proj"], x, res=x)
                ops.layernorm_f16x2(x, hbuf, blk["n2"][0], blk["n2"][1], 1e-6, blk["fc1"].in_exp)
                ops.conv_f16x2(hbuf, blk["fc1"], mid, act="gelu", out_exp=blk["fc2"].in_exp)
                ops.conv_f16x2(mid, blk["fc2"], x, res=x)
            elif self.split3:
                ops.layernorm_split3(x, hbuf, blk["n1"][0], blk["n1"][1], 1e-6)
                ops.conv_split3(hbuf, blk["qkv"], qkv)
                ops.vit_attention(qkv, att, B, S, self.heads)
                ops.conv_split3(att, blk["proj"], x, res=x)
                ops.layernorm_split3(x, hbuf, blk["n2"][0], blk["n2"][1], 1e-6)
                ops.conv_split3(hbuf, blk["fc1"], mid, act="gelu")
                ops.conv_split3(mid, blk["fc2"], x, res=x)
            else:
                ops.layernorm(x, hbuf, blk["n1"][0], blk["n1"][1], 1e-6)
                ops.conv(hbuf, blk["qkv"], qkv)
                ops.vit_attention(qkv, att, B, S, self.heads)
                ops.conv(att, blk["proj"], x, res=x)
                ops.layernorm(x, hbuf, blk["n2"][0], blk["n2"][1], 1e-6)
                ops.conv(hbuf, blk["fc1"], mid, act="gelu")
                ops.conv(mid, blk["fc2"], x, res=x)
            if taps is not None and i in (0, self.depth - 1):
                taps[f"vit_block{i}"] = x.view(B, S, D).clone()
            if i >= self.depth - 4:
                f = ops.empty((B, self.th, self.tw, D), dt, dev)
                ops.layernorm(x, f.view(B * T, D), self.norm[0], self.norm[1], 1e-6, batches=B, in_rows_per_batch=S,
                              in_row_offset=1, out_rows_per_batch=T)
                feats.append(f)
        return feats

    def forward(self, ops, img, taps=None, vit_feats=None):
        dt, dev = self.dtype, self.device
        B = img.shape[0]
        th, tw, C = self.th, self.tw, self.C
        feats = self.vit(ops, img, taps) if vit_feats is None else vit_feats
        if taps is not None:
            for i, f in enumerate(feats):
                taps[f"vit_out{i}"] = f
        maps = []
        for i, f in enumerate(feats):
            p = ops.empty((B, th, tw, self.projects[i].cout), dt, dev)
            ops.conv(f, self.projects[i], p)
            if i == 0:
                y = ops.empty((B, th * 4, tw * 4, self.oc[0]), dt, dev)
                ops.conv(p, self.up4, y)
            elif i == 1:
                y = ops.empty((B, th * 2, tw * 2, self.oc[1]), dt, dev)
                ops.conv(p, self.up2, y)
            elif i == 2:
                y = p
            else:
                y = ops.empty((B, (th + 1) // 2, (tw + 1) // 2, self.oc[3]), dt, dev)
                ops.conv(p, self.down2, y, stride=2, pad=1)
            maps.append(y)
        rn = []
        for i in range(4):
            y = ops.empty(maps[i].shape[:3] + (C,), dt, dev)
            ops.conv(maps[i], self.rn[i], y, pad=1)
            rn.append(y)
        r4 = self._refine(ops, 4, rn[3], None, rn[2].shape[1:3])
        r3 = self._refine(ops, 3, r4, rn[2], rn[1].shape[1:3])
        r2 = self._refine(ops, 2, r3, rn[1], rn[0].shape[1:3])
        r1 = self._refine(ops, 1, r2, rn[0], (rn[0].shape[1] * 2, rn[0].shape[2] * 2))
        o1 = ops.empty(r1.shape[:3] + (self.oc1.cout,), dt, dev)
        ops.conv(r1, self.oc1, o1, pad=1)
        H, W = th * 14, tw * 14
        o1u = ops.empty((B, H, W, self.oc1.cout), dt, dev)
        ops.resize(o1, o1u)
        clb = self.head.new_clb_buffer(ops, B, H, W)
        out_conv = clb[..., 0:32]
        ops.conv(o1u, self.oc2a, out_conv, pad=1, act="relu")
        ops.conv(out_conv, self.oc2b, clb[..., 32 + self.head.emb:], act="relu")
        x_d0 = ops.empty(rn[3].shape[:3] + (C,), dt, dev)
        ops.conv(rn[3], self.conv2, x_d0)
        if taps is not None:
            taps.update(dpt_layer1_rn=rn[0], dpt_layer4_rn=rn[3], rel_depth=clb[..., 32 + self.head.emb:33 + self.head.emb])
        depth = self.head.run(ops, x_d0, [r4, r3, r2, r1], clb, taps)
        return depth, [x_d0, r4, r3, r2, r1, out_conv]


def _accepts_dtype(fn):
    import inspect
    try:
        ps = inspect.signature(fn).parameters
    except (TypeError, ValueError):
        return False
    return "dtype" in ps or any(p.kind == p.VAR_KEYWORD for p in ps.values())


class ExternalCoreBranchNet:

    def __init__(self, sd, prefix, bcfg, process_shape, dtype, device, provider):
        if provider is None:
            raise NotImplementedError(
                "branch type 'ZoeDepth' needs a relative-depth core: the MiDaS/BEiT encoder is an un-vendored torch.hub "
                "repository (midas.py:340).  Pass core_providers=(coarse, fine) to PatchFusion or call set_core_providers().")
        self.dtype, self.device, self.provider = dtype, device, provider
        self.C = branch_channels(bcfg)
        self.H, self.W = process_shape
        self.conv2 = pk.pack_conv(sd[prefix + "conv2.weight"], sd[prefix + "conv2.bias"], dtype=dtype).to(device)
        self.head = BinsHead(sd, prefix, self.C, bcfg, dtype, device, with_rel=True)

    def forward(self, ops, img, taps=None):
        dt, dev = self.dtype, self.device
        if hasattr(self.provider, "forward_nhwc"):
            B, _, H, W = img.shape
            clb = self.head.new_clb_buffer(ops, B, H, W)
            if dt == F32:
                _, feats = self.provider.forward_nhwc(ops, img, out_conv=clb[..., :32], rel=clb[..., 32 + self.head.emb:])
            elif _accepts_dtype(self.provider.forward_nhwc):
                _, feats = self.provider.forward_nhwc(ops, img, out_conv=clb[..., :32], rel=clb[..., 32 + self.head.emb:], dtype=dt)
            else:
                raise NotImplementedError(f"this relative-depth core's forward_nhwc takes no dtype: it runs in float32 only (compute_dtype='fp32'), not {dt}")
            btl, blocks = feats[0], feats[1:5]
            x_d0 = ops.empty(btl.shape[:3] + (self.C,), dt, dev)
            ops.conv(btl, self.conv2, x_d0)
            depth = self.head.run(ops, x_d0, blocks, clb, taps)
            return depth, [x_d0] + blocks + [clb[..., :32]]
        rel, feats = self.provider(img)
        assert len(feats) == 6, "provider must return [btlnck, x_block0..3, out_conv]"
        nhwc = [f.detach().to(dev).permute(0, 2, 3, 1).contiguous().to(dt) for f in feats]
        btl, blocks, outc = nhwc[0], nhwc[1:5], nhwc[5]
        B, H, W = rel.shape
        clb = self.head.new_clb_buffer(ops, B, H, W)
        ops.copy_channels(outc, clb[..., :32])
        tail = torch.zeros((B, H, W, 8), dtype=dt, device=dev)
        tail[..., 0] = rel.detach().to(device=dev, dtype=dt)
        clb[..., 32 + self.head.emb:] = tail
        x_d0 = ops.empty(btl.shape[:3] + (self.C,), dt, dev)
        ops.conv(btl, self.conv2, x_d0)
        depth = self.head.run(ops, x_d0, blocks, clb, taps)
        return depth, [x_d0] + blocks + [clb[..., :32]]


class G2LNet:
    DEPTH = [4, 4, 3, 3, 2, 2]
    HEADS = [32, 32, 16, 16, 8, 8]

    def __init__(self, sd, gcfg, dtype, device, prefix="guided_fusion."):
        self.dtype, self.device = dtype, device
        from .spec import GF_DEFAULT_IN_CHANNELS
        ch = list(gcfg.get("in_channels", GF_DEFAULT_IN_CHANNELS))[::-1]
        self.levels = []
        for i, C in enumerate(ch):
            g = f"{prefix}g2l_list.{i}."
            blocks = []
            for j in range(self.DEPTH[i]):
                b = f"{g}g2l_layer.blocks.{j}."

                def pc(name):
                    return pk.pack_conv(sd[b + name + ".weight"], sd[b + name + ".bias"], dtype=dtype).to(device)
                blocks.append(dict(n1=(_g(sd, b + "norm1.weight", device), _g(sd, b + "norm1.bias", device)),
                                   n2=(_g(sd, b + "norm2.weight", device), _g(sd, b + "norm2.bias", device)),
                                   qkv=pc("attn.qkv"), proj=pc("attn.proj"), fc1=pc("mlp.fc1"), fc2=pc("mlp.fc2"),
                                   bias_table=_g(sd, b + "attn.relative_position_bias_table", device),
                                   shift=0 if j % 2 == 0 else 6))
            self.levels.append(dict(C=C, heads=self.HEADS[i], blocks=blocks,
                                    ape=_g(sd, g + "absolute_pos_embed", device)[0],
                                    norm=(_g(sd, g + "g2l_layer_norm.weight", device), _g(sd, g + "g2l_layer_norm.bias", device))))

    def forward_level(self, ops, i, feat):
        dt, dev = self.dtype, self.device
        lv = self.levels[i]
        B, H, W, C = feat.shape
        Hp, Wp = int(math.ceil(H / 12)) * 12, int(math.ceil(W / 12)) * 12
        nt = B * Hp * Wp
        x = ops.empty((B, H, W, C), dt, dev)
        ops.copy_channels(feat, x)
        ops.add_rowwise(x.view(B, H * W, C), lv["ape"])
        xw = ops.empty((nt, C), dt, dev)
        qkv = ops.empty((nt, 3 * C), dt, dev)
        ao = ops.empty((nt, C), dt, dev)
        pr = ops.empty((nt, C), dt, dev)
        hbuf = ops.empty((B * H * W, C), dt, dev)
        mid = ops.empty((B * H * W, 4 * C), dt, dev)
        for blk in lv["blocks"]:
            ops.swin_ln_partition(x, xw, blk["n1"][0], blk["n1"][1], 1e-5, blk["shift"])
            ops.conv(xw, blk["qkv"], qkv)
            ops.swin_window_attention(qkv, ao, blk["bias_table"], B, Hp, Wp, C, lv["heads"], blk["shift"])
            ops.conv(ao, blk["proj"], pr)
            x2 = ops.empty((B, H, W, C), dt, dev)
            ops.swin_unpartition_add(pr, x, x2, blk["shift"])
            x = x2
            xf = x.view(B * H * W, C)
            ops.layernorm(xf, hbuf, blk["n2"][0], blk["n2"][1], 1e-5)
            ops.conv(hbuf, blk["fc1"], mid, act="gelu")
            ops.conv(mid, blk["fc2"], xf, res=xf)
        out = ops.empty((B, H, W, C), dt, dev)
        ops.layernorm(x.view(B * H * W, C), out.view(B * H * W, C), lv["norm"][0], lv["norm"][1], 1e-5)
        return out

    def forward(self, ops, coarse_feats):
        return [self.forward_level(ops, i, f) for i, f in enumerate(coarse_feats)]


class FusionNet:

    def __init__(self, sd, cfg, dtype, device):
        self.dtype, self.device = dtype, device
        fb = cfg["fine_branch"]
        self.C = branch_channels(fb)
        self.ps = tuple(cfg["patch_process_shape"])
        self.sizes = pyramid_sizes(self.ps, fb["type"])[::-1]
        self.ch = [self.C] * 5 + [32]
        g = "guided_fusion."

        def pc(name, **kw):
            return pk.pack_conv(sd[name + ".weight"], sd.get(name + ".bias"), dtype=dtype, **kw).to(device)

        def bn(name):
            return tuple(sd[f"{name}.{k}"] for k in ("weight", "bias", "running_mean", "running_var"))

        self.fconv = [pc(f"fusion_conv_list.{i}") for i in range(6)]

        def dcbn(name, **kw):
            return (pc(name + ".double_conv.0", bn=bn(name + ".double_conv.1"), **kw),
                    pc(name + ".double_conv.3", bn=bn(name + ".double_conv.4")))

        def dcwobn(name):
            return (pc(name + ".double_conv.0"), pc(name + ".double_conv.2"))

        self.inc = dcbn(g + "inc", cin_total=8)
        self.down = [dcbn(f"{g}down_conv_list.{i}.maxpool_conv.1") for i in range(5)]
        self.upc = [dcwobn(f"{g}up_conv_list.{i}.conv") for i in range(5)]
        self.convs = [dcwobn(f"{g}convs.{i}") for i in range(6)]
        self.head = BinsHead(sd, "", self.C, cfg["coarse_branch"], dtype, device, with_rel=False,
                             min_depth=cfg["min_depth"], max_depth=cfg["max_depth"])

    def forward(self, ops, crops, rois, fine_depth, fine_feats, coarse_depth, coarse_feats, g2l, taps=None):
        dt, dev = self.dtype, self.device
        B = crops.shape[0]
        H, W = self.ps
        ch, sizes = self.ch, self.sizes
        cd_roi = ops.empty((B, 1, H, W), F32, dev)
        ops.roi_align_depth(coarse_depth, rois, cd_roi, 1.0)
        begin = getattr(ops, "cmax_begin", None)
        chain = getattr(ops, "conv_chain", None)

        def cm_kw(cm, c0=None, c1=None):
            return {} if cm is None else {"cmax": cm[c0:c1]}

        def conv_pair(x, c0, t, c1, y, cm, cm_y=None):
            if chain is not None:
                kw = {} if cm is None and cm_y is None else dict(cmax_in=cm, cmax_out=cm_y)
                return chain(x, c0, t, c1, y, dict(pad=1, act="relu"), dict(pad=1, act="relu"), **kw)
            ops.conv(x, c0, t, pad=1, act="relu")
            ops.conv(t, c1, y, pad=1, act="relu")
            return y

        guide = []
        for i in range(6):
            h, w = sizes[i]
            cat = ops.empty((B, h, w, 2 * ch[i]), dt, dev)
            gc = ops.empty((B, h, w, ch[i]), dt, dev)
            cm = begin(cat, self.fconv[i], gc, "cat", pad=1) if begin is not None else None
            ops.roi_align(coarse_feats[i], rois, cat[..., :ch[i]], h / H, **cm_kw(cm, 0, ch[i]))
            ops.copy_channels(fine_feats[i], cat[..., ch[i]:], **cm_kw(cm, ch[i], 2 * ch[i]))
            ops.conv(cat, self.fconv[i], gc, pad=1, **({} if cm is None else {"cmax_in": cm}))
            guide.append(gc)
        inp = ops.empty((B, H, W, 8), dt, dev)
        ops.pack_fusion_input(cd_roi, fine_depth, crops, inp)
        u5 = ops.empty((B, H, W, ch[5] + 2 * ch[4]), dt, dev)
        t = ops.empty((B, H, W, 32), dt, dev)
        ops.conv(inp, self.inc[0], t, pad=1, act="relu")
        e = u5[..., :32]
        ops.conv(t, self.inc[1], e, pad=1, act="relu")
        enc = [e]
        for i in range(5):
            _, hh, ww, cc = enc[-1].shape
            mp = ops.empty((B, hh // 2, ww // 2, cc), dt, dev)
            ops.maxpool2(enc[-1], mp)
            c0, c1 = self.down[i]
            t = ops.empty((B, hh // 2, ww // 2, c0.cout), dt, dev)
            ops.conv(mp, c0, t, pad=1, act="relu")
            e = ops.empty((B, hh // 2, ww // 2, c1.cout), dt, dev)
            ops.conv(t, c1, e, pad=1, act="relu")
            enc.append(e)
        enc = enc[::-1]
        clb = self.head.new_clb_buffer(ops, B, H, W)
        fused, temp = [], None
        for i in range(6):
            h, w = sizes[i]
            c = ch[i]
            v = ops.empty((B, h, w, 2 * c), dt, dev)
            tv_shape = (B, h, w, self.convs[i][0].cout)
            cmv = begin(v, self.convs[i][0], ops.empty(tv_shape, dt, dev), "v", pad=1, act="relu") if begin is not None else None
            if i == 0:
                ops.resize(enc[0], v[..., :c], **cm_kw(cmv, 0, c))
            else:
                cp = ch[i - 1]
                u = u5 if i == 5 else ops.empty((B, h, w, c + 2 * cp), dt, dev)
                c0, c1 = self.upc[i - 1]
                t = ops.empty((B, h, w, c0.cout), dt, dev)
                cmu = begin(u, c0, t, "u", pad=1, act="relu") if begin is not None else None
                if i < 5:
                    ops.resize_concat([enc[i], temp, guide[i - 1]], u, **cm_kw(cmu))
                else:
                    if cmu is not None:
                        ops.absmax(u[..., :c], cmu[:c])
                    ops.resize_concat([temp, guide[i - 1]], u[..., c:], **cm_kw(cmu, c))
                conv_pair(u, c0, t, c1, v[..., :c], cmu, None if cmv is None else cmv[:c])
                t = None
            ops.roi_align(g2l[i], rois, v[..., c:], h / H, **cm_kw(cmv, c, 2 * c))
            c0, c1 = self.convs[i]
            tv = ops.empty(tv_shape, dt, dev)
            temp = clb[..., :32] if i == 5 else ops.empty((B, h, w, c1.cout), dt, dev)
            conv_pair(v, c0, tv, c1, temp, cmv)
            fused.append(temp)
            if taps is not None:
                taps[f"gf_out{i}"] = temp
        return self.head.run(ops, fused[0], fused[1:5], clb, taps)
```

### patchfusion_amd/hip_ops.py

```python
import ctypes as C

import torch

from . import _lib
from ._lib import ConvParams, check
from .packing import PackedConv, winograd_applies

_L = _lib.load()

ACT = {"none": 0, None: 0, "relu": 1, "gelu": 2, "softplus": 3}


def _stream():
    return C.c_void_p(torch.cuda.current_stream().cuda_stream)


def _p(t):
    if t is None:
        return None
    if not t.is_cuda:
        raise _lib.PfError("patchfusion_amd.hip_ops: tensor is not on the GPU (there is no CPU path)")
    if t.device.index != torch.cuda.current_device():
        raise _lib.PfError(f"patchfusion_amd.hip_ops: tensor lives on cuda:{t.device.index} but the current device is "
                           f"cuda:{torch.cuda.current_device()} (wrap the call in torch.cuda.device(...))")
    return C.c_void_p(t.data_ptr())


def _dt(t):
    if t.dtype == torch.float32:
        return 0
    if t.dtype == torch.bfloat16:
        return 1
    raise _lib.PfError(f"unsupported dtype {t.dtype}")


def _as4(t):
    if t.dim() == 2:
        return t.unsqueeze(0).unsqueeze(0)
    if t.dim() == 3:
        return t.unsqueeze(0)
    return t


def _ld(t):
    t = _as4(t)
    B, H, W, Cc = t.shape
    assert t.stride(3) == 1, "channel stride must be 1"
    ld = t.stride(2) if W > 1 else (t.stride(1) if H > 1 else max(Cc, t.stride(2)))
    if W > 1 and H > 1:
        assert t.stride(1) == W * ld, "rows must be dense"
    if B > 1:
        assert t.stride(0) == H * W * ld, "batches must be dense"
    return ld


_ENV = {}


def _env(name, default):
    v = _ENV.get(name)
    if v is None:
        import os
        v = _ENV[name] = os.environ.get(name, default)
    return v


def refresh_env():
    _ENV.clear()
    _CONV_CACHE.clear()


_CONV_CACHE = {}


def _bf16_pp_enabled():
    return _env("PF_BF16_PP", "0") == "1"


def _conv1x1_split3_wanted(M, pw):
    mode = _env("PF_CONV1X1_SPLIT3", "1")
    if mode == "0":
        return False
    if mode == "2":
        return True
    tiles = -(-M // 64) * -(-pw.cout // 128)
    return tiles >= 512 and pw.cout >= 64


def conv1x1_split3_layout_ok(pw, x_ptr, x_ld, y_ptr, y_ld, res_ptr=None, res_ld=0, res2_ptr=None, res2_ld=0):
    if pw.w3 is None or pw.cin % 32 or pw.cout % 4 or x_ld < pw.cin or y_ld < pw.cout:
        return False
    ptrs = [x_ptr, y_ptr, pw.w3.data_ptr()] + [t.data_ptr() for t in (pw.bias, pw.scale) if t is not None]
    lds = [x_ld, y_ld]
    for ptr, ld in ((res_ptr, res_ld), (res2_ptr, res2_ld)):
        if ptr is not None:
            ptrs.append(ptr)
            lds.append(ld)
    return all(v % 16 == 0 for v in ptrs) and all(v % 4 == 0 for v in lds)


def _split3_three_step(pw):
    return pw.wino_u3 is not None and _env("PF_WINO_SPLIT3", "1") != "0"


def _wino_f16x2_enabled():
    return _env("PF_WINO_F16X2", "1") != "0"


def _fused_wanted(B, H, W, pw):
    mode = _env("PF_WINO_FUSED", "1")
    if mode == "0":
        return False
    if mode == "2":
        return True
    th, tw = -(-H // 4), -(-W // 4)
    nsuper = B * min(-(-th // 4) * -(-tw // 8), -(-th // 8) * -(-tw // 4))
    if pw.wino_u is None:
        many_out = False
    elif _split3_three_step(pw):
        many_out = pw.cout >= 256
    else:
        many_out = pw.cin >= 768 and pw.cout >= 768
    return nsuper * -(-pw.cout // 64) >= 512 and not many_out


_WS = {}
_WS16 = {}


def _workspace(device, nV, nM):
    key = (device.index, torch.cuda.current_stream().cuda_stream)
    v, m = _WS.get(key, (None, None))
    if v is None or v.numel() < nV or m is None or m.numel() < nM:
        _WS.pop(key, None)
        if v is None or v.numel() < nV:
            v = None
            v = torch.empty(nV, dtype=torch.float32, device=device)
        if m is None or m.numel() < nM:
            m = None
            m = torch.empty(nM, dtype=torch.float32, device=device)
        _WS[key] = (v, m)
    return v, m


def _f16x2_scratch(device, nbytes):
    key = (device.index, torch.cuda.current_stream().cuda_stream)
    t = _WS16.get(key)
    if t is None or t.numel() < nbytes:
        _WS16.pop(key, None)
        t = None
        t = _WS16[key] = torch.empty(nbytes, dtype=torch.uint8, device=device)
    return t


_WSCMAX = {}


def _cmax_buffer(device, n, slot="t"):
    key = (device.index, torch.cuda.current_stream().cuda_stream, slot)
    t = _WSCMAX.get(key)
    if t is None or t.numel() < n:
        t = _WSCMAX[key] = torch.empty(max(n, 1024), dtype=torch.int32, device=device)
    return t


def _cmax_handover_enabled():
    return _env("PF_WINO_F16X2_N256", "1") not in ("0", "2")


def _cmax_ptr(cmax, n):
    if cmax is None:
        return None
    assert cmax.dtype == torch.int32 and cmax.dim() == 1 and cmax.stride(0) == 1 and cmax.numel() >= n, (cmax.dtype, cmax.shape, n)
    return _p(cmax)


def release_workspaces():
    _WS.clear()
    _WS16.clear()
    _WSCMAX.clear()
    _CONV_CACHE.clear()


def workspace_bytes():
    return sum(v.numel() * 4 + m.numel() * 4 for v, m in _WS.values()) + sum(t.numel() for t in _WS16.values())


def _fused_group():
    return ((int(_env("PF_WINO_GS", "8")) & 0xffff) | (int(_env("PF_WINO_SHAPE", "0")) << 16)
            | (int(_env("PF_WINO_DBG", "0")) << 20))


def wino3_window(B, H, W, pw):
    T = B * -(-H // 4) * -(-W // 4)
    per_tile = 36 * (pw.cin * 6 + pw.cout * 4)
    cap = float(_env("PF_WS_CAP_GB", "2.5")) * 2 ** 30
    window = max(int(cap // per_tile) // 192 * 192, 192)
    if window >= T:
        window = -(-T // 8) * 8
    nwin = -(-T // window)
    return window, nwin, (36 * window * pw.cin * 3 + 1) // 2, 36 * window * pw.cout


def _align16(*ts):
    return tuple(None if t is None else t.data_ptr() % 16 for t in ts)


class HipOps:
    name = "hip"

    @staticmethod
    def empty(shape, dtype, device):
        return torch.empty(shape, dtype=dtype, device=device)

    @staticmethod
    def zeros(shape, dtype, device):
        return torch.zeros(shape, dtype=dtype, device=device)

    @staticmethod
    def _conv_plan(x, pw, y, stride, pad, act, relu_in, res, res2, direct, given=False):
        x4, y4 = _as4(x), _as4(y)
        B, H, W, _ = x4.shape
        OH = (H + 2 * pad - pw.KH) // stride + 1
        OW = (W + 2 * pad - pw.KW) // stride + 1
        s = pw.shuffle
        assert y4.shape[0] == B and y4.shape[1] == OH * s and y4.shape[2] == OW * s, (x4.shape, y4.shape, OH, OW, s)
        assert x4.shape[3] >= pw.cin and y4.shape[3] >= pw.cout // (s * s), (x4.shape, y4.shape, pw.cin, pw.cout)
        p = ConvParams()
        p.x, p.x_ld, p.B, p.H, p.W, p.Cin = x4.data_ptr(), _ld(x4), B, H, W, pw.cin
        p.w, p.w_rows, p.Kpad = pw.w.data_ptr(), pw.w.shape[0], pw.w.shape[1]
        p.bias = pw.bias.data_ptr() if pw.bias is not None else None
        p.scale = pw.scale.data_ptr() if pw.scale is not None else None
        p.res = res.data_ptr() if res is not None else None
        p.res_ld = _ld(res) if res is not None else 0
        p.res2 = res2.data_ptr() if res2 is not None else None
        p.res2_ld = _ld(res2) if res2 is not None else 0
        p.y, p.y_ld, p.OH, p.OW, p.Cout = y4.data_ptr(), _ld(y4), OH, OW, pw.cout
        p.KH, p.KW, p.stride, p.pad = pw.KH, pw.KW, stride, pad
        p.act, p.relu_in = ACT[act], int(bool(relu_in))
        p.dtype = _dt(x4)
        assert pw.w.dtype == x4.dtype, "weights must be packed in the activation dtype"
        p.out_f32 = int(y4.dtype == torch.float32 and x4.dtype != torch.float32)
        p.shuffle = s
        p.korder = pw.korder
        for t in (x4, y4, pw.w, res, res2):
            _p(t)
        f32_io = y4.dtype == torch.float32 and (res is None or res.dtype == torch.float32) and (res2 is None or res2.dtype == torch.float32)
        if (x4.dtype == torch.bfloat16 and pw.KH == 1 and pw.KW == 1 and stride == 1 and pad == 0 and s == 1 and not relu_in and not direct and
                B * H * W >= 2048 and pw.cin % 64 == 0 and pw.cin >= 512 and pw.cout >= 512 and _bf16_pp_enabled()):
            return "pp", p, None
        if (pw.w3 is not None and x4.dtype == torch.float32 and f32_io and stride == 1 and pad == 0 and s == 1 and not direct and
                conv1x1_split3_layout_ok(pw, p.x, p.x_ld, p.y, p.y_ld, p.res, p.res_ld, p.res2, p.res2_ld) and _conv1x1_split3_wanted(B * H * W, pw)):
            return "s3_1x1", p, (_p(pw.w3), pw.w3.shape[2])
        wino = winograd_applies(pw, B * H * W, stride, pad, act) and not direct
        if wino and pw.wino_up is not None and _fused_wanted(B, H, W, pw) and _L.pf_conv_winograd_fused_supported(C.byref(p)):
            assert f32_io
            return "fused", p, (_p(pw.wino_up), pw.wino_up.shape[0], _fused_group())
        if wino and pw.wino_u is not None:
            m = pw.wino_m
            T = B * -(-H // m) * -(-W // m)
            a2 = (m + 2) ** 2
            assert f32_io
            if m == 4 and _split3_three_step(pw):
                window, _, nV, nM = wino3_window(B, H, W, pw)
                rows, kpad = pw.wino_u.shape[1], pw.wino_u.shape[2]
                if _wino_f16x2_enabled() and _L.pf_conv_winograd_f16x2_supported_ex(C.byref(p), rows, kpad, window, int(bool(given))):
                    return "wino3h", p, (_p(pw.wino_u), rows, kpad, 36 * window * pw.cin, nM, window, _L.pf_wino_f16x2_scratch_bytes(pw.cin, rows))
                return "wino3", p, (_p(pw.wino_u3), pw.wino_u3.shape[3], pw.wino_u3.shape[2] * 32, nV, nM, window)
            return "wino", p, (m, _p(pw.wino_u), pw.wino_u.shape[1], pw.wino_u.shape[2], a2 * T * pw.cin, a2 * T * pw.cout)
        return "direct", p, None

    @staticmethod
    def _conv_exec(route, p, extra, device, cmax_in=None, cmax_out=None, cmax_out_relu=False):
        assert (cmax_in is None or route == "wino3h") and (cmax_out is None or route in ("wino3", "wino3h")), route
        if route == "direct":
            check(_L.pf_conv(C.byref(p), _stream()), "pf_conv")
        elif route == "s3_1x1":
            check(_L.pf_conv1x1_split3(C.byref(p), extra[0], extra[1], _stream()), "pf_conv1x1_split3")
        elif route == "fused":
            check(_L.pf_conv_winograd_fused(C.byref(p), extra[0], extra[1], extra[2], _stream()), "pf_conv_winograd_fused")
        elif route == "wino3":
            V, Mw = _workspace(device, extra[3], extra[4])
            if cmax_out is not None:
                check(_L.pf_conv_winograd_split3_windowed_ex(C.byref(p), extra[0], extra[1], extra[2], C.c_void_p(V.data_ptr()), C.c_void_p(Mw.data_ptr()),
                                                             extra[5], C.c_void_p(cmax_out.data_ptr()), int(cmax_out_relu), _stream()),
                      "pf_conv_winograd_split3_windowed_ex")
                return
            check(_L.pf_conv_winograd_split3_windowed(C.byref(p), extra[0], extra[1], extra[2], C.c_void_p(V.data_ptr()), C.c_void_p(Mw.data_ptr()),
                                                      extra[5], _stream()), "pf_conv_winograd_split3_windowed")
        elif route == "wino3h":
            V, Mw = _workspace(device, extra[3], extra[4])
            S = _f16x2_scratch(device, extra[6])
            if cmax_in is not None or cmax_out is not None:
                check(_L.pf_conv_winograd_f16x2_windowed_ex(C.byref(p), extra[0], extra[1], extra[2], C.c_void_p(V.data_ptr()), C.c_void_p(Mw.data_ptr()),
                                                            C.c_void_p(S.data_ptr()), extra[5], None if cmax_in is None else C.c_void_p(cmax_in.data_ptr()),
                                                            None if cmax_out is None else C.c_void_p(cmax_out.data_ptr()), int(cmax_out_relu), _stream()),
                      "pf_conv_winograd_f16x2_windowed_ex")
                return
            check(_L.pf_conv_winograd_f16x2_windowed(C.byref(p), extra[0], extra[1], extra[2], C.c_void_p(V.data_ptr()), C.c_void_p(Mw.data_ptr()),
                                                     C.c_void_p(S.data_ptr()), extra[5], _stream()), "pf_conv_winograd_f16x2_windowed")
        elif route == "wino":
            V, Mw = _workspace(device, extra[4], extra[5])
            check(_L.pf_conv_winograd(C.byref(p), extra[0], extra[1], extra[2], extra[3], C.c_void_p(V.data_ptr()), C.c_void_p(Mw.data_ptr()), _stream()),
                  "pf_conv_winograd")
        else:
            check(_L.pf_gemm_bf16_pp(C.byref(p), _stream()), "pf_gemm_bf16_pp")

    @staticmethod
    def conv(x, pw: PackedConv, y, stride=1, pad=0, act=None, relu_in=False, res=None, res2=None, _timed=None, _direct=None, cmax_in=None):
        if _timed is None and _direct is None:
            ent = HipOps._conv_plan_cached(x, pw, y, stride, pad, act, relu_in, res, res2, cmax_in is not None)
            if cmax_in is not None and ent[1] != "wino3h":
                raise _lib.PfError("conv: cmax_in given to a layer that does not run the fp16x2 Winograd form (ask cmax_begin first)")
            HipOps._conv_exec(ent[1], ent[2], ent[3], x.device, cmax_in=cmax_in)
            return y
        assert cmax_in is None
        route, p, extra = HipOps._conv_plan(x, pw, y, stride, pad, act, relu_in, res, res2, _direct)
        return HipOps._conv_uncached(route, p, extra, x, y, _timed)

    @staticmethod
    def cmax_begin(x, pw, y, slot, stride=1, pad=0, act=None, relu_in=False, res=None, res2=None):
        if relu_in or not _cmax_handover_enabled() or x.dtype != torch.float32 or x.shape[-1] != pw.cin:
            return None
        ent = HipOps._conv_plan_cached(x, pw, y, stride, pad, act, relu_in, res, res2, True)
        if ent[1] != "wino3h":
            return None
        cm = _cmax_buffer(x.device, pw.cin, slot)[:pw.cin]
        check(_L.pf_zero_u32(_p(cm), pw.cin, _stream()), "pf_zero_u32")
        return cm

    @staticmethod
    def absmax(x, cmax):
        x4 = _as4(x)
        B, H, W, Cc = x4.shape
        assert x4.dtype == torch.float32
        check(_L.pf_wino_absmax(_p(x4), _ld(x4), B * H * W, Cc, 0, _cmax_ptr(cmax, Cc), _stream()), "pf_wino_absmax")

    @staticmethod
    def conv_chain(x, pw1, t, pw2, y, kw1, kw2, cmax_in=None, cmax_out=None):
        def plan(a, pw, b, kw, given):
            return HipOps._conv_plan_cached(a, pw, b, kw.get("stride", 1), kw.get("pad", 0), kw.get("act"), kw.get("relu_in", False), kw.get("res"),
                                            kw.get("res2"), given)
        e1 = plan(x, pw1, t, kw1, cmax_in is not None)
        if cmax_in is not None and e1[1] != "wino3h":
            raise _lib.PfError("conv_chain: cmax_in given to a layer that does not run the fp16x2 Winograd form (ask cmax_begin first)")
        e2 = None
        if e1[1] in ("wino3", "wino3h") and t.shape[-1] == pw1.cout == pw2.cin and _cmax_handover_enabled():
            e2 = plan(t, pw2, y, kw2, True)
        three = ("wino3", "wino3h")
        if e2 is not None and e2[1] == "wino3h":
            cm = _cmax_buffer(x.device, pw1.cout)
            HipOps._conv_exec(e1[1], e1[2], e1[3], x.device, cmax_in=cmax_in, cmax_out=cm, cmax_out_relu=bool(kw2.get("relu_in", False)))
            HipOps._conv_exec(e2[1], e2[2], e2[3], x.device, cmax_in=cm, cmax_out=cmax_out)
        else:
            e2 = plan(t, pw2, y, kw2, False)
            HipOps._conv_exec(e1[1], e1[2], e1[3], x.device, cmax_in=cmax_in)
            HipOps._conv_exec(e2[1], e2[2], e2[3], x.device, cmax_out=cmax_out if e2[1] in three else None)
            if cmax_out is not None and e2[1] not in three:
                HipOps.absmax(y[..., :pw2.cout], cmax_out)
        return y

    @staticmethod
    def _conv_plan_cached(x, pw, y, stride, pad, act, relu_in, res, res2, given=False):
        key = (id(pw), x.shape, x.stride(), y.shape, y.stride(), stride, pad, act, relu_in, x.dtype, y.dtype, x.device,
               None if res is None else (res.shape, res.stride(), res.dtype), None if res2 is None else (res2.shape, res2.stride(), res2.dtype),
               _align16(x, y, res, res2), bool(given))
        ent = _CONV_CACHE.get(key)
        if ent is None or ent[0] is not pw:
            if len(_CONV_CACHE) > 4096:
                _CONV_CACHE.clear()
            ent = (pw,) + HipOps._conv_plan(x, pw, y, stride, pad, act, relu_in, res, res2, None, given)
            _CONV_CACHE[key] = ent
        else:
            p = ent[2]
            p.x, p.y = x.data_ptr(), y.data_ptr()
            if res is not None:
                p.res = res.data_ptr()
            if res2 is not None:
                p.res2 = res2.data_ptr()
        return ent

    @staticmethod
    def _conv_uncached(route, p, extra, x, y, _timed):
        if _timed is None:
            HipOps._conv_exec(route, p, extra, x.device)
            return y
        if route == "direct":
            ms = C.c_float(0)
            check(_L.pf_conv_timed(C.byref(p), int(_timed), C.byref(ms), _stream()), "pf_conv_timed")
            return ms.value
        if route == "fused":
            ms = C.c_float(0)
            check(_L.pf_conv_winograd_fused_timed(C.byref(p), extra[0], extra[1], extra[2], int(_timed), C.byref(ms), _stream()),
                  "pf_conv_winograd_fused_timed")
            return ms.value
        HipOps._conv_exec(route, p, extra, x.device)
        e0, e1 = torch.cuda.Event(enable_timing=True), torch.cuda.Event(enable_timing=True)
        e0.record()
        for _ in range(int(_timed)):
            HipOps._conv_exec(route, p, extra, x.device)
        e1.record()
        e1.synchronize()
        return e0.elapsed_time(e1) / int(_timed)

    @staticmethod
    def gemm_planes_split3(V3, U3, Mw, T, cin, cout, iters=None):
        P = V3.shape[1]
        kmaj = V3.dim() == 5
        assert V3.dim() == U3.dim() and V3.dtype == U3.dtype == torch.bfloat16 and Mw.dtype == torch.float32 and U3.shape[:2] == (3, P)
        assert tuple(V3.shape) == ((3, P, cin // 32, T, 32) if kmaj else (3, P, T, cin)) and (U3.shape[2] * 32 if kmaj else U3.shape[3]) == cin
        assert V3.is_contiguous() and U3.is_contiguous() and Mw.is_contiguous() and Mw.numel() >= P * T * cout
        p = ConvParams()
        p.x, p.x_ld, p.B, p.H, p.W, p.Cin = V3.data_ptr(), cin, 1, 1, T, cin
        p.w, p.w_rows, p.Kpad = U3.data_ptr(), U3.shape[3] if kmaj else U3.shape[2], cin
        p.korder = 6 if kmaj else 0
        p.y, p.y_ld, p.OH, p.OW, p.Cout = Mw.data_ptr(), cout, 1, T, cout
        p.KH = p.KW = p.stride = 1
        p.act, p.shuffle, p.dtype, p.out_f32, p.batch = 0, 1, 1, 1, P
        p.x_bstride, p.w_bstride = V3.stride(0), U3.stride(0)
        for t in (V3, U3, Mw):
            _p(t)
        if iters is None:
            check(_L.pf_gemm_split3(C.byref(p), _stream()), "pf_gemm_split3")
            return Mw
        ms = C.c_float(0)
        check(_L.pf_gemm_split3_timed(C.byref(p), int(iters), C.byref(ms), _stream()), "pf_gemm_split3_timed")
        return ms.value

    @staticmethod
    def gemm_planes_split3_timed(V3, U3, Mw, T, cin, cout, iters):
        return HipOps.gemm_planes_split3(V3, U3, Mw, T, cin, cout, iters)

    @staticmethod
    def gemm_planes_timed(V, U, Mw, planes, T, cin, cout, iters):
        assert V.dtype == U.dtype == Mw.dtype == torch.float32 and V.numel() >= planes * T * cin and Mw.numel() >= planes * T * cout
        p = ConvParams()
        p.x, p.x_ld, p.B, p.H, p.W, p.Cin = V.data_ptr(), cin, 1, 1, T, cin
        p.w, p.w_rows, p.Kpad = U.data_ptr(), U.shape[1], U.shape[2]
        p.y, p.y_ld, p.OH, p.OW, p.Cout = Mw.data_ptr(), cout, 1, T, cout
        p.KH = p.KW = p.stride = 1
        p.shuffle, p.dtype = 1, 0
        p.batch, p.x_bstride, p.w_bstride, p.y_bstride = planes, T * cin, U.shape[1] * U.shape[2], T * cout
        for t in (V, U, Mw):
            _p(t)
        ms = C.c_float(0)
        check(_L.pf_conv_timed(C.byref(p), int(iters), C.byref(ms), _stream()), "pf_conv_timed")
        return ms.value

    @staticmethod
    def split3(x, y3):
        assert x.dtype == torch.float32 and y3.dtype == torch.bfloat16 and y3.dim() == 3 and y3.shape[0] == 3 and y3.is_contiguous()
        M, K = x.shape
        check(_L.pf_split3(_p(x), x.stride(0), _p(y3), y3.stride(1), y3.stride(0), M, K, _stream()), "pf_split3")
        return y3

    @staticmethod
    def _conv_split3_plan(x3, pw, y, act, res, res2):
        assert x3.dtype == torch.bfloat16 and x3.shape[0] == 3 and pw.w.dtype == torch.bfloat16
        split_out = y.dtype == torch.bfloat16
        p = ConvParams()
        korder = 0
        if x3.dim() == 4:
            assert x3.is_contiguous() and x3.shape[3] == 32 and x3.shape[1] * 32 == pw.cin
            M = x3.shape[2]
            p.x, p.x_ld = x3.data_ptr(), pw.cin
            korder |= 2
        else:
            assert x3.dim() == 3 and x3.stride(2) == 1 and x3.shape[2] >= pw.cin
            M = x3.shape[1]
            p.x, p.x_ld = x3.data_ptr(), x3.stride(1)
        p.B, p.H, p.W, p.Cin = 1, 1, M, pw.cin
        p.x_bstride = x3.stride(0)
        if pw.w.dim() == 4:
            assert pw.w.is_contiguous() and pw.w.shape[1] * 32 == pw.cin
            p.w, p.w_rows, p.Kpad, p.w_bstride = pw.w.data_ptr(), pw.w.shape[2], pw.cin, pw.w.stride(0)
            korder |= 4
        else:
            p.w, p.w_rows, p.Kpad, p.w_bstride = pw.w.data_ptr(), pw.w.shape[1], pw.w.shape[2], pw.w.stride(0)
        p.bias = pw.bias.data_ptr() if pw.bias is not None else None
        p.scale = pw.scale.data_ptr() if pw.scale is not None else None
        p.res = res.data_ptr() if res is not None else None
        p.res_ld = res.stride(-2) if res is not None else 0
        p.res2 = res2.data_ptr() if res2 is not None else None
        p.res2_ld = res2.stride(-2) if res2 is not None else 0
        if split_out and y.dim() == 4:
            assert y.is_contiguous() and tuple(y.shape) == (3, pw.cout // 32, M, 32) and pw.cout % 32 == 0
            p.y, p.y_ld, p.y_bstride, p.out_f32 = y.data_ptr(), pw.cout, y.stride(0), 0
            korder |= 8
        elif split_out:
            assert y.dim() == 3 and y.shape[0] == 3 and y.shape[1] == M and y.stride(2) == 1
            p.y, p.y_ld, p.y_bstride, p.out_f32 = y.data_ptr(), y.stride(1), y.stride(0), 0
        else:
            assert y.dtype == torch.float32 and y.stride(-1) == 1
            p.y, p.y_ld, p.out_f32 = y.data_ptr(), y.stride(-2), 1
        p.OH, p.OW, p.Cout = 1, M, pw.cout
        p.KH = p.KW = p.stride = 1
        p.act, p.shuffle, p.dtype, p.korder = ACT[act], 1, 1, korder
        for t in (x3, y, pw.w, res, res2):
            _p(t)
        for t in (res, res2):
            assert t is None or (t.dtype == torch.float32 and t.shape[-1] >= pw.cout and t.shape[-2] == M), "residuals are float32 [M, >= N]"
        assert y.dim() == 4 or (y.shape[-1] >= pw.cout and y.shape[-2] == M)
        return p

    @staticmethod
    def conv_split3(x3, pw: PackedConv, y, act=None, res=None, res2=None, _timed=None):
        key = (id(pw), x3.shape, x3.stride(), y.shape, y.stride(), y.dtype, act, x3.device,
               None if res is None else (res.shape, res.stride()), None if res2 is None else (res2.shape, res2.stride()))
        ent = _CONV_CACHE.get(key)
        if ent is None or ent[0] is not pw:
            if len(_CONV_CACHE) > 4096:
                _CONV_CACHE.clear()
            ent = (pw, HipOps._conv_split3_plan(x3, pw, y, act, res, res2))
            _CONV_CACHE[key] = ent
        else:
            p = ent[1]
            p.x, p.y = x3.data_ptr(), y.data_ptr()
            if res is not None:
                p.res = res.data_ptr()
            if res2 is not None:
                p.res2 = res2.data_ptr()
        p = ent[1]
        if _timed is not None:
            ms = C.c_float(0)
            check(_L.pf_gemm_split3_timed(C.byref(p), int(_timed), C.byref(ms), _stream()), "pf_gemm_split3_timed")
            return ms.value
        check(_L.pf_gemm_split3(C.byref(p), _stream()), "pf_gemm_split3")
        return y

    @staticmethod
    def _conv_f16x2_plan(x2, pw, y, act, res, res2, out_exp):
        assert x2.dtype == pw.w.dtype == torch.float16 and x2.dim() == 4 and x2.shape[0] == 2 and x2.shape[3] == 32 and x2.is_contiguous()
        assert x2.shape[1] * 32 == pw.cin and pw.w.dim() == 4 and pw.w.is_contiguous() and pw.col_exp is not None
        M = x2.shape[2]
        p = ConvParams()
        p.x, p.x_ld, p.x_bstride = x2.data_ptr(), pw.cin, x2.stride(0)
        p.B, p.H, p.W, p.Cin = 1, 1, M, pw.cin
        p.w, p.w_rows, p.Kpad, p.w_bstride = pw.w.data_ptr(), pw.w.shape[2], pw.cin, pw.w.stride(0)
        p.bias = pw.bias.data_ptr() if pw.bias is not None else None
        p.scale = pw.scale.data_ptr() if pw.scale is not None else None
        p.col_exp = _p(pw.col_exp)
        p.res = res.data_ptr() if res is not None else None
        p.res_ld = res.stride(-2) if res is not None else 0
        p.res2 = res2.data_ptr() if res2 is not None else None
        p.res2_ld = res2.stride(-2) if res2 is not None else 0
        korder = 6
        if y.dtype == torch.float16 and y.dim() == 3:
            assert y.shape[0] == 2 and y.shape[1] == M and y.stride(2) == 1 and y.shape[2] >= pw.cout and y.stride(1) % 4 == 0
            assert out_exp is not None and out_exp.dtype == torch.int32 and out_exp.numel() >= pw.cout
            p.y, p.y_ld, p.y_bstride, p.out_f32, p.out_exp = y.data_ptr(), y.stride(1), y.stride(0), 0, _p(out_exp)
            korder |= 32
        elif y.dtype == torch.float16:
            assert y.is_contiguous() and tuple(y.shape) == (2, pw.cout // 32, M, 32) and pw.cout % 32 == 0
            assert out_exp is not None and out_exp.dtype == torch.int32 and out_exp.numel() >= pw.cout
            p.y, p.y_ld, p.y_bstride, p.out_f32, p.out_exp = y.data_ptr(), pw.cout, y.stride(0), 0, _p(out_exp)
            korder |= 16
        elif y.dtype == torch.bfloat16:
            assert y.dim() == 3 and y.shape[0] == 3 and y.shape[1] == M and y.stride(2) == 1 and y.shape[2] >= pw.cout
            p.y, p.y_ld, p.y_bstride, p.out_f32 = y.data_ptr(), y.stride(1), y.stride(0), 0
        else:
            assert y.dtype == torch.float32 and y.stride(-1) == 1 and y.shape[-2] == M and y.shape[-1] >= pw.cout
            p.y, p.y_ld, p.out_f32 = y.data_ptr(), y.stride(-2), 1
        p.OH, p.OW, p.Cout = 1, M, pw.cout
        p.KH = p.KW = p.stride = 1
        p.act, p.shuffle, p.dtype, p.korder = ACT[act], 1, 1, korder
        for t in (x2, y, pw.w, res, res2):
            _p(t)
        for t in (res, res2):
            assert t is None or (t.dtype == torch.float32 and t.shape[-1] >= pw.cout and t.shape[-2] == M), "residuals are float32 [M, >= N]"
        return p

    @staticmethod
    def conv_f16x2(x2, pw: PackedConv, y, act=None, res=None, res2=None, out_exp=None):
        key = ("f16x2", id(pw), x2.shape, y.shape, y.stride(), y.dtype, act, x2.device,
               None if res is None else (res.shape, res.stride()), None if res2 is None else (res2.shape, res2.stride()),
               None if out_exp is None else out_exp.data_ptr())
        ent = _CONV_CACHE.get(key)
        if ent is None or ent[0] is not pw:
            if len(_CONV_CACHE) > 4096:
                _CONV_CACHE.clear()
            ent = (pw, HipOps._conv_f16x2_plan(x2, pw, y, act, res, res2, out_exp))
            _CONV_CACHE[key] = ent
        else:
            p = ent[1]
            p.x, p.y = x2.data_ptr(), y.data_ptr()
            if res is not None:
                p.res = res.data_ptr()
            if res2 is not None:
                p.res2 = res2.data_ptr()
        check(_L.pf_gemm_f16x2(C.byref(ent[1]), _stream()), "pf_gemm_f16x2")
        return y

    @staticmethod
    def patch_im2col(img, out):
        B, _, H, W = img.shape
        assert img.dtype == torch.float32 and img.is_contiguous()
        check(_L.pf_patch_im2col(_p(img), B, H, W, _p(out), out.stride(0), _dt(out), _stream()), "pf_patch_im2col")

    @staticmethod
    def assemble_tokens(emb, tokens, cls, pos):
        B, S, D = tokens.shape
        assert emb.is_contiguous() and tokens.is_contiguous()
        check(_L.pf_assemble_tokens(_p(emb), _p(tokens), _p(cls), _p(pos), B, S, D, _dt(tokens), _stream()), "pf_assemble_tokens")

    @staticmethod
    def layernorm(x, y, g, b, eps, batches=1, in_rows_per_batch=None, in_row_offset=0, out_rows_per_batch=None):
        D = x.shape[-1]
        rows = x.numel() // D
        if in_rows_per_batch is None:
            in_rows_per_batch = out_rows_per_batch = rows
            batches = 1
        check(_L.pf_layernorm(_p(x), x.stride(-2), _p(y), y.stride(-2), _p(g), _p(b), float(eps), batches, in_rows_per_batch,
                              in_row_offset, out_rows_per_batch, D, _dt(x), _stream()), "pf_layernorm")

    @staticmethod
    def layernorm_split3(x, y3, g, b, eps):
        assert x.dtype == torch.float32 and y3.dtype == torch.bfloat16 and y3.shape[0] == 3
        M, D = x.shape
        if y3.dim() == 4:
            assert y3.is_contiguous() and tuple(y3.shape) == (3, D // 32, M, 32)
            check(_L.pf_layernorm_split3(_p(x), x.stride(0), _p(y3), D, y3.stride(0), 1, _p(g), _p(b), float(eps), M, D, _stream()),
                  "pf_layernorm_split3")
            return y3
        assert y3.dim() == 3 and y3.stride(2) == 1 and y3.shape[1] == M and y3.shape[2] == D
        check(_L.pf_layernorm_split3(_p(x), x.stride(0), _p(y3), y3.stride(1), y3.stride(0), 0, _p(g), _p(b), float(eps), M, D, _stream()),
              "pf_layernorm_split3")
        return y3

    @staticmethod
    def layernorm_f16x2(x, y2, g, b, eps, in_exp):
        assert x.dtype == torch.float32 and x.stride(-1) == 1 and y2.dtype == torch.float16 and in_exp.dtype == torch.int32
        M, D = x.shape
        assert y2.is_contiguous() and tuple(y2.shape) == (2, D // 32, M, 32) and in_exp.numel() == D
        check(_L.pf_layernorm_f16x2(_p(x), x.stride(0), _p(y2), _p(in_exp), _p(g), _p(b), float(eps), M, D, _stream()), "pf_layernorm_f16x2")
        return y2

    @staticmethod
    def vit_attention(qkv, out, B, S, heads):
        kmaj = int(out.dim() == 4)
        if qkv.dim() == 3:
            D = qkv.shape[2] // 3
            assert qkv.dtype == out.dtype == torch.bfloat16 and tuple(qkv.shape) == (3, B * S, 3 * D)
            assert tuple(out.shape) == ((3, D // 32, B * S, 32) if kmaj else (3, B * S, D))
            assert D == heads * 64 and qkv.is_contiguous() and out.is_contiguous()
            if _env("PF_ATTN_V2", "1") != "0":
                check(_L.pf_vit_attention_split3_v2(_p(qkv), qkv.stride(0), _p(out), out.stride(0), kmaj, B, S, heads, int(_env("PF_ATTN_QW", "0")),
                                                    int(_env("PF_ATTN_SCHED", "0")), _stream()), "pf_vit_attention_split3_v2")
                return
            check(_L.pf_vit_attention_split3(_p(qkv), qkv.stride(0), _p(out), out.stride(0), kmaj, B, S, heads, _stream()), "pf_vit_attention_split3")
            return
        D = qkv.shape[1] // 3
        assert D == heads * 64 and qkv.is_contiguous() and out.is_contiguous()
        if qkv.dtype == torch.float32 and out.dtype == torch.bfloat16:
            assert tuple(out.shape) == ((3, D // 32, B * S, 32) if kmaj else (3, B * S, D))
            check(_L.pf_vit_attention_qkv_split3(_p(qkv), _p(out), out.stride(0), kmaj, B, S, heads, _stream()), "pf_vit_attention_qkv_split3")
            return
        if qkv.dtype == torch.float32 and _env("PF_ATTN_QKV", "1") != "0":
            check(_L.pf_vit_attention_qkv(_p(qkv), _p(out), B, S, heads, 0, _stream()), "pf_vit_attention_qkv")
            return
        Sp = (S + 63) // 64 * 64
        q = torch.empty((B, heads, S, 64), dtype=qkv.dtype, device=qkv.device)
        k = torch.empty_like(q)
        vt = torch.empty((B, heads, 64, Sp), dtype=qkv.dtype, device=qkv.device)
# ... 346 lines not shown
```

Before: 109.3 patches/s.

## Fuse bilinear resize-concat into the fp16x2 Winograd input transform

```diff
diff --git a/include/pf_hip.h b/include/pf_hip.h
--- a/include/pf_hip.h
+++ b/include/pf_hip.h
@@ -47,6 +47,9 @@
                                     void* stream);
 int pf_conv_winograd_f16x2_windowed_ex(const pf_conv_params* p, const void* U, int u_rows, int u_kpad, void* V2, void* M, void* scratch, long window,
                                        const void* cmax_in, void* cmax_out, int cmax_out_relu, void* stream);
+int pf_conv_winograd_f16x2_windowed_src(const pf_conv_params* p, const void* U, int u_rows, int u_kpad, void* V2, void* M, void* scratch, long window,
+                                        const void* const* xs, const int* lds, const int* Hs, const int* Ws, const int* Cs, int nsrc, int src_dtype,
+                                        const void* cmax_in, void* cmax_out, int cmax_out_relu, void* stream);
 int pf_conv_winograd_split3_windowed_ex(const pf_conv_params* p, const void* U3, int u_rows, int u_kpad, void* V3, void* M, long window, void* cmax_out,
                                         int cmax_out_relu, void* stream);
 int pf_wino_absmax(const void* x, int x_ld, long P, int C, int relu_in, void* cmax, void* stream);
diff --git a/patchfusion_amd/_lib.py b/patchfusion_amd/_lib.py
--- a/patchfusion_amd/_lib.py
+++ b/patchfusion_amd/_lib.py
@@ -54,6 +54,8 @@
     "pf_conv_winograd_split3_windowed": [C.POINTER(ConvParams), vp, ci, ci, vp, vp, C.c_long, vp],
     "pf_conv_winograd_f16x2_windowed": [C.POINTER(ConvParams), vp, ci, ci, vp, vp, vp, C.c_long, vp],
     "pf_conv_winograd_f16x2_windowed_ex": [C.POINTER(ConvParams), vp, ci, ci, vp, vp, vp, C.c_long, vp, vp, ci, vp],
+    "pf_conv_winograd_f16x2_windowed_src": [C.POINTER(ConvParams), vp, ci, ci, vp, vp, vp, C.c_long, C.POINTER(vp), C.POINTER(ci), C.POINTER(ci),
+                                            C.POINTER(ci), C.POINTER(ci), ci, ci, vp, vp, ci, vp],
     "pf_conv_winograd_split3_windowed_ex": [C.POINTER(ConvParams), vp, ci, ci, vp, vp, C.c_long, vp, ci, vp],
     "pf_wino_absmax": [vp, ci, cl, ci, ci, vp, vp],
     "pf_gemm_f16x2_points": [C.POINTER(ConvParams), vp, ci, vp],
diff --git a/patchfusion_amd/csrc/imageops.hip b/patchfusion_amd/csrc/imageops.hip
--- a/patchfusion_amd/csrc/imageops.hip
+++ b/patchfusion_amd/csrc/imageops.hip
@@ -14,25 +14,6 @@
 }
 inline int ok() { return hipGetLastError() == hipSuccess ? PF_OK : PF_ERR_LAUNCH; }
 
-struct Lerp {
-  int i0, i1;
-  float l0, l1;
-};
-__device__ __forceinline__ Lerp ac_coord(int dst, float scale, int in) {
-#pragma clang fp contract(off)
-  const float src = scale * dst;
-  Lerp r;
-  r.i0 = (int)src;
-  r.i1 = r.i0 + (r.i0 < in - 1 ? 1 : 0);
-  r.l1 = src - r.i0;
-  r.l0 = 1.0f - r.l1;
-  return r;
-}
-__device__ __forceinline__ float bilerp(const Lerp& ly, const Lerp& lx, float v00, float v01, float v10, float v11) {
-#pragma clang fp contract(off)
-  return ly.l0 * (lx.l0 * v00 + lx.l1 * v01) + ly.l1 * (lx.l0 * v10 + lx.l1 * v11);
-}
-inline float ac_scale(int in, int out) { return out > 1 ? (float)(in - 1) / (float)(out - 1) : 0.f; }
 
 template <typename T>
 __device__ __forceinline__ void ld8x(const void* p, long off, int f32, float (&v)[8]) {
@@ -78,11 +59,6 @@
   }
 }
 
-struct ResizeSrc {
-  const void* x;
-  int ld, H, W, C;
-  float sh, sw;
-};
 template <typename T>
 __global__ void resize_concat_kernel(ResizeSrc s0, ResizeSrc s1, ResizeSrc s2, int nsrc, int B, void* __restrict__ y, int y_ld,
                                      int OH, int OW) {
diff --git a/patchfusion_amd/csrc/pf_common.h b/patchfusion_amd/csrc/pf_common.h
--- a/patchfusion_amd/csrc/pf_common.h
+++ b/patchfusion_amd/csrc/pf_common.h
@@ -138,6 +138,39 @@
   return base + idx;
 }
 
+struct Lerp {
+  int i0, i1;
+  float l0, l1;
+};
+__device__ __forceinline__ Lerp ac_coord(int dst, float scale, int in) {
+#pragma clang fp contract(off)
+  const float src = scale * dst;
+  Lerp r;
+  r.i0 = (int)src;
+  r.i1 = r.i0 + (r.i0 < in - 1 ? 1 : 0);
+  r.l1 = src - r.i0;
+  r.l0 = 1.0f - r.l1;
+  return r;
+}
+__device__ __forceinline__ float hlerp(const Lerp& lx, float v0, float v1) {
+#pragma clang fp contract(off)
+  return lx.l0 * v0 + lx.l1 * v1;
+}
+__device__ __forceinline__ float vlerp(const Lerp& ly, float h0, float h1) {
+#pragma clang fp contract(off)
+  return ly.l0 * h0 + ly.l1 * h1;
+}
+__device__ __forceinline__ float bilerp(const Lerp& ly, const Lerp& lx, float v00, float v01, float v10, float v11) {
+  return vlerp(ly, hlerp(lx, v00, v01), hlerp(lx, v10, v11));
+}
+inline float ac_scale(int in, int out) { return out > 1 ? (float)(in - 1) / (float)(out - 1) : 0.f; }
+
+struct ResizeSrc {
+  const void* x;
+  int ld, H, W, C;
+  float sh, sw;
+};
+
 #define PF_OK 0
 #define PF_ERR_ARG 1
 #define PF_ERR_LAUNCH 2
diff --git a/patchfusion_amd/csrc/wino_f16x2.hip b/patchfusion_amd/csrc/wino_f16x2.hip
--- a/patchfusion_amd/csrc/wino_f16x2.hip
+++ b/patchfusion_amd/csrc/wino_f16x2.hip
@@ -1,19 +1,9 @@
 #include <climits>
 #include "pf_common.h"
+#include "wino_f16x2_common.h"
 #include "../../include/pf_hip.h"
 
 namespace {
-
-__device__ __forceinline__ int clog2(float a) {
-  int e;
-  const float f = frexpf(a, &e);
-  return f == 0.5f ? e - 1 : e;
-}
-__device__ __forceinline__ int chan_exp(unsigned mb) { return (mb == 0u || mb >= 0x7f800000u) ? 0 : clog2(__uint_as_float(mb)) - 8; }
-
-__device__ __forceinline__ uint32_t pack_h2(_Float16 a, _Float16 b) {
-  return (uint32_t)__builtin_bit_cast(uint16_t, a) | ((uint32_t)__builtin_bit_cast(uint16_t, b) << 16);
-}
 
 __global__ __launch_bounds__(256) void wino_absmax_kernel(const float* __restrict__ x, int x_ld, long P, int C, int relu_in, long R,
                                                           unsigned* __restrict__ cmax) {
@@ -76,16 +66,6 @@
   if (lane == 0) fexp[pt * rows + n] = f;
 }
 
-__device__ __forceinline__ void bt6(float (&d)[6]) {
-  const float o0 = 4.f * d[0] - 5.f * d[2] + d[4];
-  const float o1 = -4.f * (d[1] + d[2]) + d[3] + d[4];
-  const float o2 = 4.f * (d[1] - d[2]) - d[3] + d[4];
-  const float o3 = -2.f * d[1] - d[2] + 2.f * d[3] + d[4];
-  const float o4 = 2.f * d[1] - d[2] - 2.f * d[3] + d[4];
-  const float o5 = 4.f * d[1] - 5.f * d[3] + d[5];
-  d[0] = o0; d[1] = o1; d[2] = o2; d[3] = o3; d[4] = o4; d[5] = o5;
-}
-
 __global__ __launch_bounds__(512) void wino_input_f16x2_kernel(const float* __restrict__ x, int x_ld, int B, int H, int W, int C, int relu_in,
                                                                const unsigned* __restrict__ cmax, uint16_t* __restrict__ V, int TH, int TW, long total,
                                                                long tile0, long T) {
@@ -114,44 +94,7 @@
         d[i][j][0] = v.x; d[i][j][1] = v.y; d[i][j][2] = v.z; d[i][j][3] = v.w;
       }
     }
-#pragma unroll
-    for (int e = 0; e < 4; ++e) {
-#pragma unroll
-      for (int j = 0; j < A; ++j) {
-        float col[A];
-#pragma unroll
-        for (int i = 0; i < A; ++i) col[i] = d[i][j][e];
-        bt6(col);
-#pragma unroll
-        for (int i = 0; i < A; ++i) d[i][j][e] = col[i];
-      }
-#pragma unroll
-      for (int i = 0; i < A; ++i) {
-        float row[A];
-#pragma unroll
-        for (int j = 0; j < A; ++j) row[j] = d[i][j][e];
-        bt6(row);
-#pragma unroll
-        for (int j = 0; j < A; ++j) d[i][j][e] = row[j];
-      }
-    }
-    const size_t plane = (size_t)T * C;
-    uint16_t* o = V + ((size_t)(c4 >> 3) * T + tile) * 32 + (c4 & 7) * 4;
-#pragma unroll
-    for (int i = 0; i < A; ++i)
-#pragma unroll
-      for (int j = 0; j < A; ++j) {
-        _Float16 h[4], l[4];
-#pragma unroll
-        for (int e = 0; e < 4; ++e) {
-          const float v = ldexpf(d[i][j][e], ne[e]);
-          h[e] = (_Float16)v;
-          l[e] = (_Float16)(v - (float)h[e]);
-        }
-        uint16_t* q = o + (size_t)(i * A + j) * plane;
-        *reinterpret_cast<uint2*>(q) = make_uint2(pack_h2(h[0], h[1]), pack_h2(h[2], h[3]));
-        *reinterpret_cast<uint2*>(q + (size_t)A * A * plane) = make_uint2(pack_h2(l[0], l[1]), pack_h2(l[2], l[3]));
-      }
+    f16x2_transform_store(d, ne, V, tile, T, C, c4);
   }
 }
 
diff --git a/patchfusion_amd/csrc/wino_f16x2_common.h b/patchfusion_amd/csrc/wino_f16x2_common.h
--- /dev/null
+++ b/patchfusion_amd/csrc/wino_f16x2_common.h
@@ -0,0 +1,69 @@
+#pragma once
+#include "pf_common.h"
+
+namespace {
+
+__device__ __forceinline__ int clog2(float a) {
+  int e;
+  const float f = frexpf(a, &e);
+  return f == 0.5f ? e - 1 : e;
+}
+__device__ __forceinline__ int chan_exp(unsigned mb) { return (mb == 0u || mb >= 0x7f800000u) ? 0 : clog2(__uint_as_float(mb)) - 8; }
+
+__device__ __forceinline__ uint32_t pack_h2(_Float16 a, _Float16 b) {
+  return (uint32_t)__builtin_bit_cast(uint16_t, a) | ((uint32_t)__builtin_bit_cast(uint16_t, b) << 16);
+}
+
+__device__ __forceinline__ void bt6(float (&d)[6]) {
+  const float o0 = 4.f * d[0] - 5.f * d[2] + d[4];
+  const float o1 = -4.f * (d[1] + d[2]) + d[3] + d[4];
+  const float o2 = 4.f * (d[1] - d[2]) - d[3] + d[4];
+  const float o3 = -2.f * d[1] - d[2] + 2.f * d[3] + d[4];
+  const float o4 = 2.f * d[1] - d[2] - 2.f * d[3] + d[4];
+  const float o5 = 4.f * d[1] - 5.f * d[3] + d[5];
+  d[0] = o0; d[1] = o1; d[2] = o2; d[3] = o3; d[4] = o4; d[5] = o5;
+}
+
+__device__ __forceinline__ void f16x2_transform_store(float (&d)[6][6][4], const int (&ne)[4], uint16_t* __restrict__ V, long tile, long T, int C, int c4) {
+  constexpr int A = 6;
+#pragma unroll
+  for (int e = 0; e < 4; ++e) {
+#pragma unroll
+    for (int j = 0; j < A; ++j) {
+      float col[A];
+#pragma unroll
+      for (int i = 0; i < A; ++i) col[i] = d[i][j][e];
+      bt6(col);
+#pragma unroll
+      for (int i = 0; i < A; ++i) d[i][j][e] = col[i];
+    }
+#pragma unroll
+    for (int i = 0; i < A; ++i) {
+      float row[A];
+#pragma unroll
+      for (int j = 0; j < A; ++j) row[j] = d[i][j][e];
+      bt6(row);
+#pragma unroll
+      for (int j = 0; j < A; ++j) d[i][j][e] = row[j];
+    }
+  }
+  const size_t plane = (size_t)T * C;
+  uint16_t* o = V + ((size_t)(c4 >> 3) * T + tile) * 32 + (c4 & 7) * 4;
+#pragma unroll
+  for (int i = 0; i < A; ++i)
+#pragma unroll
+    for (int j = 0; j < A; ++j) {
+      _Float16 h[4], l[4];
+#pragma unroll
+      for (int e = 0; e < 4; ++e) {
+        const float v = ldexpf(d[i][j][e], ne[e]);
+        h[e] = (_Float16)v;
+        l[e] = (_Float16)(v - (float)h[e]);
+      }
+      uint16_t* q = o + (size_t)(i * A + j) * plane;
+      *reinterpret_cast<uint2*>(q) = make_uint2(pack_h2(h[0], h[1]), pack_h2(h[2], h[3]));
+      *reinterpret_cast<uint2*>(q + (size_t)A * A * plane) = make_uint2(pack_h2(l[0], l[1]), pack_h2(l[2], l[3]));
+    }
+}
+
+}
diff --git a/patchfusion_amd/csrc/wino_f16x2_src.hip b/patchfusion_amd/csrc/wino_f16x2_src.hip
--- /dev/null
+++ b/patchfusion_amd/csrc/wino_f16x2_src.hip
@@ -0,0 +1,129 @@
+#include <cstdlib>
+#include "pf_common.h"
+#include "wino_f16x2_common.h"
+#include "../../include/pf_hip.h"
+
+namespace {
+
+template <int G>
+__global__ __launch_bounds__(512) void wino_input_f16x2_src_kernel(ResizeSrc s0, ResizeSrc s1, ResizeSrc s2, int B, int H, int W, int C,
+                                                                   const unsigned* __restrict__ cmax, uint16_t* __restrict__ V, int TH, int TW,
+                                                                   long total, long tile0, long T) {
+  constexpr int MT = 4, A = 6;
+  static_assert(A % G == 0, "column groups");
+  const int nkc = C >> 5;
+  for (long idx = (long)blockIdx.x * blockDim.x + threadIdx.x; idx < total; idx += (long)gridDim.x * blockDim.x) {
+    const long w64 = idx >> 6;
+    const long tile = (w64 / nkc) * 8 + ((idx >> 3) & 7);
+    const int kc = (int)(w64 % nkc);
+    const int c4 = kc * 8 + (int)(idx & 7);
+    if (tile >= T) continue;
+    const long gt = tile + tile0;
+    const int tx = (int)(gt % TW), ty = (int)((gt / TW) % TH), b = (int)(gt / ((long)TW * TH));
+    const uint4 mb = *reinterpret_cast<const uint4*>(cmax + c4 * 4);
+    const int ne[4] = {-chan_exp(mb.x), -chan_exp(mb.y), -chan_exp(mb.z), -chan_exp(mb.w)};
+    const int ch0 = __builtin_amdgcn_readfirstlane(kc) * 32;
+    const int si = ch0 < s0.C ? 0 : (ch0 < s0.C + s1.C ? 1 : 2);
+    ResizeSrc s;
+    s.x = si == 0 ? s0.x : (si == 1 ? s1.x : s2.x);
+    s.ld = si == 0 ? s0.ld : (si == 1 ? s1.ld : s2.ld);
+    s.H = si == 0 ? s0.H : (si == 1 ? s1.H : s2.H);
+    s.W = si == 0 ? s0.W : (si == 1 ? s1.W : s2.W);
+    s.sh = si == 0 ? s0.sh : (si == 1 ? s1.sh : s2.sh);
+    s.sw = si == 0 ? s0.sw : (si == 1 ? s1.sw : s2.sw);
+    const int cs = c4 * 4 - (si == 0 ? 0 : (si == 1 ? s0.C : s0.C + s1.C));
+    const float* __restrict__ sx = static_cast<const float*>(s.x) + (long)b * s.H * s.W * s.ld + cs;
+    float d[A][A][4];
+#pragma unroll
+    for (int g = 0; g < A; g += G) {
+      Lerp lx[G];
+      int o0[G], o1[G];
+      bool in[G];
+#pragma unroll
+      for (int j = 0; j < G; ++j) {
+        const int xx = tx * MT - 1 + g + j;
+        in[j] = (unsigned)xx < (unsigned)W;
+        lx[j] = ac_coord(in[j] ? xx : 0, s.sw, s.W);
+        o0[j] = lx[j].i0 * s.ld;
+        o1[j] = lx[j].i1 * s.ld;
+      }
+      float ha[G][4], hb[G][4];
+      int ra = -1, rb = -1;
+      auto fetch = [&](int r, float (&h)[G][4]) __attribute__((always_inline)) {
+        const float* __restrict__ rp = sx + (long)r * s.W * s.ld;
+#pragma unroll
+        for (int j = 0; j < G; ++j) {
+          const float4 v0 = *reinterpret_cast<const float4*>(rp + o0[j]);
+          const float4 v1 = *reinterpret_cast<const float4*>(rp + o1[j]);
+          h[j][0] = hlerp(lx[j], v0.x, v1.x); h[j][1] = hlerp(lx[j], v0.y, v1.y);
+          h[j][2] = hlerp(lx[j], v0.z, v1.z); h[j][3] = hlerp(lx[j], v0.w, v1.w);
+        }
+      };
+#pragma unroll
+      for (int i = 0; i < A; ++i) {
+        const int y = ty * MT - 1 + i;
+        if ((unsigned)y < (unsigned)H) {
+          const Lerp ly = ac_coord(y, s.sh, s.H);
+          if (ly.i0 != ra) {
+            if (ly.i0 == rb) {
+#pragma unroll
+              for (int j = 0; j < G; ++j)
+#pragma unroll
+                for (int e = 0; e < 4; ++e) ha[j][e] = hb[j][e];
+            } else {
+              fetch(ly.i0, ha);
+            }
+            ra = ly.i0;
+          }
+          if (ly.i1 != rb) {
+            if (ly.i1 == ra) {
+#pragma unroll
+              for (int j = 0; j < G; ++j)
+#pragma unroll
+                for (int e = 0; e < 4; ++e) hb[j][e] = ha[j][e];
+            } else {
+              fetch(ly.i1, hb);
+            }
+            rb = ly.i1;
+          }
+#pragma unroll
+          for (int j = 0; j < G; ++j)
+#pragma unroll
+            for (int e = 0; e < 4; ++e) d[i][g + j][e] = in[j] ? vlerp(ly, ha[j][e], hb[j][e]) : 0.f;
+        } else {
+#pragma unroll
+          for (int j = 0; j < G; ++j)
+#pragma unroll
+            for (int e = 0; e < 4; ++e) d[i][g + j][e] = 0.f;
+        }
+      }
+    }
+#pragma unroll
+    for (int i = 0; i < A; ++i)
+#pragma unroll
+      for (int j = 0; j < A; ++j)
+#pragma unroll
+        for (int e = 0; e < 4; ++e) asm volatile("" : "+v"(d[i][j][e]));
+    f16x2_transform_store(d, ne, V, tile, T, C, c4);
+  }
+}
+
+}
+
+namespace pf_f16x2 {
+
+int launch_input_src(const ResizeSrc* src, int nsrc, int B, int H, int W, int C, const unsigned* cmax, void* V, int TH, int TW, long tile0, long T,
+                     hipStream_t st) {
+  static const int g = [] { const char* e = getenv("PF_WINO_SRC_G"); const int v = e ? atoi(e) : 6; return v == 2 || v == 3 ? v : 6; }();
+  const long nin = ((T + 7) / 8) * 8 * (C / 4);
+  const ResizeSrc none{};
+  const dim3 grid((unsigned)((nin + 255) / 256)), block(256);
+  uint16_t* v = static_cast<uint16_t*>(V);
+  const ResizeSrc &a = src[0], &b = nsrc > 1 ? src[1] : none, &c = nsrc > 2 ? src[2] : none;
+  if (g == 6) hipLaunchKernelGGL(wino_input_f16x2_src_kernel<6>, grid, block, 0, st, a, b, c, B, H, W, C, cmax, v, TH, TW, nin, tile0, T);
+  else if (g == 3) hipLaunchKernelGGL(wino_input_f16x2_src_kernel<3>, grid, block, 0, st, a, b, c, B, H, W, C, cmax, v, TH, TW, nin, tile0, T);
+  else hipLaunchKernelGGL(wino_input_f16x2_src_kernel<2>, grid, block, 0, st, a, b, c, B, H, W, C, cmax, v, TH, TW, nin, tile0, T);
+  return hipGetLastError() == hipSuccess ? PF_OK : PF_ERR_LAUNCH;
+}
+
+}
diff --git a/patchfusion_amd/csrc/winograd.hip b/patchfusion_amd/csrc/winograd.hip
--- a/patchfusion_amd/csrc/winograd.hip
+++ b/patchfusion_amd/csrc/winograd.hip
@@ -8,6 +8,8 @@
 int launch_input(const float* x, int x_ld, int B, int H, int W, int C, int relu_in, const unsigned* cmax, void* V, int TH, int TW, long tile0, long T,
                  hipStream_t st);
 int launch_output_cmax(const float* M, const pf_conv_params* p, int TH, int TW, long t0, long T, unsigned* cmax, int cmax_relu, hipStream_t st);
+int launch_input_src(const ResizeSrc* src, int nsrc, int B, int H, int W, int C, const unsigned* cmax, void* V, int TH, int TW, long tile0, long T,
+                     hipStream_t st);
 }
 
 namespace {
@@ -331,14 +333,15 @@
 }
 
 int run_f16x2(const pf_conv_params* p, const float* U, int u_rows, void* V2, float* M, void* scratch, long window, hipStream_t st,
-              const unsigned* cmax_in = nullptr, unsigned* cmax_out = nullptr, int cmax_relu = 0) {
+              const unsigned* cmax_in = nullptr, unsigned* cmax_out = nullptr, int cmax_relu = 0, const ResizeSrc* src = nullptr, int nsrc = 0) {
   constexpr int MT = 4;
   const bool t128 = f16x2_layer_route(p, u_rows, cmax_in != nullptr) == PF_S3_ROUTE_PERSIST128;
   const int TH = (p->H + MT - 1) / MT, TW = (p->W + MT - 1) / MT;
   const long Tall = (long)p->B * TH * TW;
   if (Tall > 0x7fffffffL) return PF_ERR_ARG;
   if (window <= 0 || window > Tall) window = Tall;
-  if (window < Tall && windows_alias(p)) return PF_ERR_ARG;
+  if (src && !cmax_in) return PF_ERR_ARG;
+  if (!src && window < Tall && windows_alias(p)) return PF_ERR_ARG;
   const F16x2Scratch sc = f16x2_scratch(scratch, p->Cin, u_rows);
   const float* x = static_cast<const float*>(p->x);
   int rc = PF_OK;
@@ -355,7 +358,8 @@
   for (long t0 = 0; t0 < Tall; t0 += window) {
     const long T = Tall - t0 < window ? Tall - t0 : window;
     const long nout = T * (p->Cout / 4);
-    rc = pf_f16x2::launch_input(x, p->x_ld, p->B, p->H, p->W, p->Cin, p->relu_in, cmax, V2, TH, TW, t0, T, st);
+    rc = src ? pf_f16x2::launch_input_src(src, nsrc, p->B, p->H, p->W, p->Cin, cmax, V2, TH, TW, t0, T, st)
+             : pf_f16x2::launch_input(x, p->x_ld, p->B, p->H, p->W, p->Cin, p->relu_in, cmax, V2, TH, TW, t0, T, st);
     if (rc != PF_OK) return rc;
     const pf_conv_params q = f16x2_points_params(p, sc.u2, u_rows, V2, M, T);
     rc = t128 ? pf_gemm_f16x2_points128(&q, sc.fexp, 0, st) : pf_gemm_f16x2_points(&q, sc.fexp, 0, st);
@@ -374,7 +378,7 @@
 }
 
 bool f16x2_args_ok(const pf_conv_params* p, int u_rows, int u_kpad, long window) {
-  if (!p || !p->x || !p->y || window < 0 || (window > 0 && window % 8)) return false;
+  if (!p || !p->y || window < 0 || (window > 0 && window % 8)) return false;
   if (p->dtype != PF_DTYPE_F32 || p->KH != 3 || p->KW != 3 || p->stride != 1 || p->pad != 1 || p->shuffle > 1 || p->scale) return false;
   if (p->OH != p->H || p->OW != p->W || p->Cin % 32 || p->Cout % 8 || p->Cin <= 0 || p->Cout <= 0 || p->Cin > 8192) return false;
   if (p->act != PF_ACT_NONE && p->act != PF_ACT_RELU) return false;
@@ -400,15 +404,41 @@
 
 extern "C" int pf_conv_winograd_f16x2_windowed(const pf_conv_params* p, const void* U, int u_rows, int u_kpad, void* V2, void* M, void* scratch,
                                                long window, void* stream) {
-  if (!U || !V2 || !M || !scratch || !f16x2_args_ok(p, u_rows, u_kpad, window)) return PF_ERR_ARG;
+  if (!U || !V2 || !M || !scratch || !f16x2_args_ok(p, u_rows, u_kpad, window) || !p->x) return PF_ERR_ARG;
   return run_f16x2(p, static_cast<const float*>(U), u_rows, V2, static_cast<float*>(M), scratch, window, ST(stream));
 }
 
 extern "C" int pf_conv_winograd_f16x2_windowed_ex(const pf_conv_params* p, const void* U, int u_rows, int u_kpad, void* V2, void* M, void* scratch,
                                                   long window, const void* cmax_in, void* cmax_out, int cmax_out_relu, void* stream) {
-  if (!U || !V2 || !M || !scratch || !f16x2_args_ok(p, u_rows, u_kpad, window) || (cmax_in && cmax_in == cmax_out)) return PF_ERR_ARG;
+  if (!U || !V2 || !M || !scratch || !f16x2_args_ok(p, u_rows, u_kpad, window) || !p->x || (cmax_in && cmax_in == cmax_out)) return PF_ERR_ARG;
   return run_f16x2(p, static_cast<const float*>(U), u_rows, V2, static_cast<float*>(M), scratch, window, ST(stream),
                    static_cast<const unsigned*>(cmax_in), static_cast<unsigned*>(cmax_out), cmax_out_relu);
+}
+
+extern "C" int pf_conv_winograd_f16x2_windowed_src(const pf_conv_params* p, const void* U, int u_rows, int u_kpad, void* V2, void* M, void* scratch,
+                                                   long window, const void* const* xs, const int* lds, const int* Hs, const int* Ws, const int* Cs, int nsrc,
+                                                   int src_dtype, const void* cmax_in, void* cmax_out, int cmax_out_relu, void* stream) {
+  if (!U || !V2 || !M || !scratch || !f16x2_args_ok(p, u_rows, u_kpad, window) || !cmax_in || cmax_in == cmax_out) return PF_ERR_ARG;
+  if (p->relu_in || src_dtype != PF_DTYPE_F32 || !xs || !lds || !Hs || !Ws || !Cs || nsrc < 1 || nsrc > 3) return PF_ERR_ARG;
+  ResizeSrc src[3] = {};
+  long csum = 0;
+  const long Tall = (long)p->B * ((p->H + 3) / 4) * ((p->W + 3) / 4);
+  const bool windows = window > 0 && window < Tall;
+  const char* y0 = static_cast<const char*>(p->y);
+  const char* y1 = y0 + ((size_t)p->B * p->H * p->W - 1) * p->y_ld * 4 + (size_t)p->Cout * 4;
+  for (int i = 0; i < nsrc; ++i) {
+    if (!xs[i] || Hs[i] <= 0 || Ws[i] <= 0 || Cs[i] <= 0 || Cs[i] % 32 || lds[i] < Cs[i] || lds[i] % 4 || reinterpret_cast<uintptr_t>(xs[i]) % 16)
+      return PF_ERR_ARG;
+    if ((long)Ws[i] * lds[i] > 0x7fffffffL) return PF_ERR_ARG;
+    const char* a0 = static_cast<const char*>(xs[i]);
+    const char* a1 = a0 + ((size_t)p->B * Hs[i] * Ws[i] - 1) * lds[i] * 4 + (size_t)Cs[i] * 4;
+    if (windows && a0 < y1 && y0 < a1) return PF_ERR_ARG;
+    src[i] = ResizeSrc{xs[i], lds[i], Hs[i], Ws[i], Cs[i], ac_scale(Hs[i], p->H), ac_scale(Ws[i], p->W)};
+    csum += Cs[i];
+  }
+  if (csum != p->Cin) return PF_ERR_ARG;
+  return run_f16x2(p, static_cast<const float*>(U), u_rows, V2, static_cast<float*>(M), scratch, window, ST(stream),
+                   static_cast<const unsigned*>(cmax_in), static_cast<unsigned*>(cmax_out), cmax_out_relu, src, nsrc);
 }
 
 extern "C" int pf_wino_absmax(const void* x, int x_ld, long P, int C, int relu_in, void* cmax, void* stream) {
diff --git a/patchfusion_amd/engine.py b/patchfusion_amd/engine.py
--- a/patchfusion_amd/engine.py
+++ b/patchfusion_amd/engine.py
@@ -549,7 +549,9 @@
             guide.append(gc)
         inp = ops.empty((B, H, W, 8), dt, dev)
         ops.pack_fusion_input(cd_roi, fine_depth, crops, inp)
-        u5 = ops.empty((B, H, W, ch[5] + 2 * ch[4]), dt, dev)
+        fuse = getattr(ops, "conv_resized", None)
+        fuse5 = fuse is not None and ops.conv_resized_wanted(B, (H, W), self.upc[4][0], dt, pad=1, act="relu")
+        u5 = ops.empty((B, H, W, ch[5] + (0 if fuse5 else 2 * ch[4])), dt, dev)
         t = ops.empty((B, H, W, 32), dt, dev)
         ops.conv(inp, self.inc[0], t, pad=1, act="relu")
         e = u5[..., :32]
@@ -578,17 +580,25 @@
                 ops.resize(enc[0], v[..., :c], **cm_kw(cmv, 0, c))
             else:
                 cp = ch[i - 1]
-                u = u5 if i == 5 else ops.empty((B, h, w, c + 2 * cp), dt, dev)
                 c0, c1 = self.upc[i - 1]
                 t = ops.empty((B, h, w, c0.cout), dt, dev)
-                cmu = begin(u, c0, t, "u", pad=1, act="relu") if begin is not None else None
-                if i < 5:
-                    ops.resize_concat([enc[i], temp, guide[i - 1]], u, **cm_kw(cmu))
-                else:
-                    if cmu is not None:
-                        ops.absmax(u[..., :c], cmu[:c])
-                    ops.resize_concat([temp, guide[i - 1]], u[..., c:], **cm_kw(cmu, c))
-                conv_pair(u, c0, t, c1, v[..., :c], cmu, None if cmv is None else cmv[:c])
+                srcs = [u5[..., :c] if i == 5 else enc[i], temp, guide[i - 1]]
+                done = None
+                if fuse is not None and (i < 5 or fuse5):
+                    done = fuse(srcs, (h, w), c0, t, "u", pad=1, act="relu", then=(c1, v[..., :c], dict(pad=1, act="relu")),
+                                cmax_out=None if cmv is None else cmv[:c])
+                if done is None:
+                    assert i < 5 or not fuse5, "the last level's concat buffer was sized for the fused up conv"
+                    u = u5 if i == 5 else ops.empty((B, h, w, c + 2 * cp), dt, dev)
+                    cmu = begin(u, c0, t, "u", pad=1, act="relu") if begin is not None else None
+                    if i < 5:
+                        ops.resize_concat(srcs, u, **cm_kw(cmu))
+                    else:
+                        if cmu is not None:
+                            ops.absmax(u[..., :c], cmu[:c])
+                        ops.resize_concat(srcs[1:], u[..., c:], **cm_kw(cmu, c))
+                    conv_pair(u, c0, t, c1, v[..., :c], cmu, None if cmv is None else cmv[:c])
+                    u = None
                 t = None
             ops.roi_align(g2l[i], rois, v[..., c:], h / H, **cm_kw(cmv, c, 2 * c))
             c0, c1 = self.convs[i]
diff --git a/patchfusion_amd/hip_ops.py b/patchfusion_amd/hip_ops.py
--- a/patchfusion_amd/hip_ops.py
+++ b/patchfusion_amd/hip_ops.py
@@ -105,6 +105,10 @@
 
 def _wino_f16x2_enabled():
     return _env("PF_WINO_F16X2", "1") != "0"
+
+
+def _resize_fuse_enabled():
+    return _env("PF_WINO_RESIZE_FUSE", "1") != "0"
 
 
 def _fused_wanted(B, H, W, pw):
@@ -344,21 +348,109 @@
         e1 = plan(x, pw1, t, kw1, cmax_in is not None)
         if cmax_in is not None and e1[1] != "wino3h":
             raise _lib.PfError("conv_chain: cmax_in given to a layer that does not run the fp16x2 Winograd form (ask cmax_begin first)")
+
+        def run1(cm, relu):
+            HipOps._conv_exec(e1[1], e1[2], e1[3], x.device, cmax_in=cmax_in, cmax_out=cm, cmax_out_relu=relu)
+        return HipOps._chain_second(run1, e1[1] in ("wino3", "wino3h"), pw1, t, pw2, y, kw2, cmax_out)
+
+    @staticmethod
+    def _chain_second(run1, first_three, pw1, t, pw2, y, kw2, cmax_out):
+        def plan(given):
+            return HipOps._conv_plan_cached(t, pw2, y, kw2.get("stride", 1), kw2.get("pad", 0), kw2.get("act"), kw2.get("relu_in", False), kw2.get("res"),
+                                            kw2.get("res2"), given)
         e2 = None
-        if e1[1] in ("wino3", "wino3h") and t.shape[-1] == pw1.cout == pw2.cin and _cmax_handover_enabled():
-            e2 = plan(t, pw2, y, kw2, True)
+        if first_three and t.shape[-1] == pw1.cout == pw2.cin and _cmax_handover_enabled():
+            e2 = plan(True)
         three = ("wino3", "wino3h")
         if e2 is not None and e2[1] == "wino3h":
-            cm = _cmax_buffer(x.device, pw1.cout)
-            HipOps._conv_exec(e1[1], e1[2], e1[3], x.device, cmax_in=cmax_in, cmax_out=cm, cmax_out_relu=bool(kw2.get("relu_in", False)))
-            HipOps._conv_exec(e2[1], e2[2], e2[3], x.device, cmax_in=cm, cmax_out=cmax_out)
+            cm = _cmax_buffer(t.device, pw1.cout)
+            run1(cm, bool(kw2.get("relu_in", False)))
+            HipOps._conv_exec(e2[1], e2[2], e2[3], t.device, cmax_in=cm, cmax_out=cmax_out)
         else:
-            e2 = plan(t, pw2, y, kw2, False)
-            HipOps._conv_exec(e1[1], e1[2], e1[3], x.device, cmax_in=cmax_in)
-            HipOps._conv_exec(e2[1], e2[2], e2[3], x.device, cmax_out=cmax_out if e2[1] in three else None)
+            e2 = plan(False)
+            run1(None, False)
+            HipOps._conv_exec(e2[1], e2[2], e2[3], t.device, cmax_out=cmax_out if e2[1] in three else None)
             if cmax_out is not None and e2[1] not in three:
                 HipOps.absmax(y[..., :pw2.cout], cmax_out)
         return y
+
+    @staticmethod
+    def _resized_plan(B, OH, OW, pw, y_ptr, y_ld, pad, act):
+        if not (_resize_fuse_enabled() and _cmax_handover_enabled() and _wino_f16x2_enabled()):
+            return None
+        if pw.w.dtype != torch.float32 or pw.shuffle != 1 or pw.KH != 3 or pw.KW != 3 or pad != 1:
+            return None
+        if not winograd_applies(pw, B * OH * OW, 1, pad, act) or pw.wino_u is None or pw.wino_m != 4 or not _split3_three_step(pw):
+            return None
+        if pw.wino_up is not None and _fused_wanted(B, OH, OW, pw):
+            return None
+        p = ConvParams()
+        p.x, p.x_ld, p.B, p.H, p.W, p.Cin = None, pw.cin, B, OH, OW, pw.cin
+        p.w, p.w_rows, p.Kpad = pw.w.data_ptr(), pw.w.shape[0], pw.w.shape[1]
+        p.bias = pw.bias.data_ptr() if pw.bias is not None else None
+        p.scale = pw.scale.data_ptr() if pw.scale is not None else None
+        p.y, p.y_ld, p.OH, p.OW, p.Cout = y_ptr, y_ld, OH, OW, pw.cout
+        p.KH, p.KW, p.stride, p.pad = 3, 3, 1, pad
+        p.act, p.relu_in, p.dtype, p.out_f32, p.shuffle, p.korder = ACT[act], 0, 0, 0, 1, pw.korder
+        window, _, _, nM = wino3_window(B, OH, OW, pw)
+        rows, kpad = pw.wino_u.shape[1], pw.wino_u.shape[2]
+        if not _L.pf_conv_winograd_f16x2_supported_ex(C.byref(p), rows, kpad, window, 1):
+            return None
+        return p, (_p(pw.wino_u), rows, kpad, 36 * window * pw.cin, nM, window, _L.pf_wino_f16x2_scratch_bytes(pw.cin, rows))
+
+    @staticmethod
+    def conv_resized_wanted(B, out_hw, pw, dtype, pad=0, act=None):
+        if dtype != torch.float32:
+            return False
+        return HipOps._resized_plan(B, out_hw[0], out_hw[1], pw, pw.w.data_ptr(), pw.cout, pad, act) is not None
+
+    @staticmethod
+    def conv_resized(srcs, out_hw, pw, y, slot, pad=0, act=None, then=None, cmax_out=None):
+        n = len(srcs)
+        OH, OW = out_hw
+        B = srcs[0].shape[0]
+        if not 1 <= n <= 3 or any(x.dim() != 4 or x.dtype != torch.float32 or x.shape[0] != B or x.shape[3] % 32 or x.data_ptr() % 16 or _ld(x) % 4
+                                  for x in srcs) or sum(x.shape[3] for x in srcs) != pw.cin:
+            return None
+        key = ("resized", id(pw), tuple((x.shape, x.stride()) for x in srcs), OH, OW, y.shape, y.stride(), pad, act, y.dtype, y.device, _align16(y))
+        ent = _CONV_CACHE.get(key)
+        if ent is None or ent[0] is not pw:
+            if len(_CONV_CACHE) > 4096:
+                _CONV_CACHE.clear()
+            y4 = _as4(y)
+            assert y4.shape[:3] == (B, OH, OW) and y4.shape[3] >= pw.cout, (y4.shape, B, OH, OW, pw.cout)
+            plan = HipOps._resized_plan(B, OH, OW, pw, _p(y4).value, _ld(y4), pad, act) if y4.dtype == torch.float32 else None
+            ent = _CONV_CACHE[key] = (pw, plan)
+        elif ent[1] is not None:
+            ent[1][0].y = y.data_ptr()
+        if ent[1] is None:
+            return None
+        p, extra = ent[1]
+        dev = y.device
+        for x in srcs:
+            _p(x)
+        cm = _cmax_buffer(dev, pw.cin, slot)[:pw.cin]
+        check(_L.pf_zero_u32(_p(cm), pw.cin, _stream()), "pf_zero_u32")
+        c0 = 0
+        for x in srcs:
+            HipOps.absmax(x, cm[c0:c0 + x.shape[3]])
+            c0 += x.shape[3]
+        ptrs = (C.c_void_p * n)(*[x.data_ptr() for x in srcs])
+        arr = lambda v: (C.c_int * n)(*v)
+        geo = (arr([_ld(x) for x in srcs]), arr([x.shape[1] for x in srcs]), arr([x.shape[2] for x in srcs]), arr([x.shape[3] for x in srcs]))
+
+        def run1(cmo, relu):
+            V, Mw = _workspace(dev, extra[3], extra[4])
+            S = _f16x2_scratch(dev, extra[6])
+            check(_L.pf_conv_winograd_f16x2_windowed_src(C.byref(p), extra[0], extra[1], extra[2], C.c_void_p(V.data_ptr()), C.c_void_p(Mw.data_ptr()),
+                                                         C.c_void_p(S.data_ptr()), extra[5], ptrs, *geo, n, 0, C.c_void_p(cm.data_ptr()),
+                                                         None if cmo is None else C.c_void_p(cmo.data_ptr()), int(relu), _stream()),
+                  "pf_conv_winograd_f16x2_windowed_src")
+        if then is None:
+            run1(cmax_out, False)
+            return y
+        pw2, y2, kw2 = then
+        return HipOps._chain_second(run1, True, pw, y, pw2, y2, kw2, cmax_out)
 
     @staticmethod
     def _conv_plan_cached(x, pw, y, stride, pad, act, relu_in, res, res2, given=False):
```

Result: no change. 109.3 patches/s (-0.0%).
